# SimonsRoad/gf-pl-slam

Hardware: AMD Instinct MI355X
Metric: stereo frames/sec (2k ORB + 500 LBD, 10 GN iters) (higher is better)
Workload: dtype f64

## Files before the change

### gf-pl-slam_amd/csrc/gfpl_abi.hip

```cpp
#include <hip/hip_runtime.h>

#include <algorithm>
#include <atomic>
#include <cmath>
#include <mutex>
#include <cstdio>
#include <cstdlib>
#include <cstring>
#include <vector>

#include "../../include/gfpl.h"
#include "gfpl_kernels.hpp"

using namespace gfpl;

#define GFPL_NEV 10

struct gfpl_ctx {
    int device = 0;
    hipStream_t stream = nullptr;
    bool own_stream = false;
    gfpl_camera cam{};
    gfpl_config cfg{};
    bool has_cam = false, has_cfg = false;
    bool timing = false;
    hipEvent_t ev[GFPL_NEV]{};
    float stage_ms[7]{};
    std::vector<gfpl_seqbatch*> sbs;
    std::atomic<int> n_detectors{0};
    std::mutex host_mu;
    char* fuse_ws = nullptr;
    size_t fuse_ws_bytes = 0;
    int* fuse_host = nullptr;
    hipEvent_t fuse_ev[2][4]{};
    bool fuse_timed[2] = {false, false};
};

struct gfpl_seqbatch {
    gfpl_ctx* ctx = nullptr;
    int B = 0, kp_cap = 0, kl_cap = 0, mpt_cap = 0, mls_cap = 0;
    void* base = nullptr;
    int64_t bytes = 0;
    DevFrame slot[2];
    int prev_slot = 0;
    bool initialized = false;
    bool has_curr = false;
    DevTrack tr{};
    DevScratch scr{};
    void* stage[2] = {nullptr, nullptr};
    size_t stage_bytes[2] = {0, 0};
    gfpl_frames stage_view[2]{};
    hipStream_t copy = nullptr;
    hipEvent_t ev_ready[2]{}, ev_free[2]{};
    bool ready_pending[2] = {false, false}, free_recorded[2] = {false, false};
    hipEvent_t ev_ticket[16]{};
    int64_t n_tickets = 0;
    int32_t* last_n_pt = nullptr;
    int32_t* last_n_ls = nullptr;
    PyrBuild* pyrb = nullptr;
    int last_cut_mode = -1;
};

struct gfpl_event {
    int device = 0;
    hipEvent_t ev = nullptr;
    int64_t records = 0;
};

int gfpl_ctx_device(const gfpl_ctx* c) { return c->device; }
void* gfpl_ctx_stream(const gfpl_ctx* c) { return (void*)c->stream; }
const gfpl_camera* gfpl_ctx_camera(const gfpl_ctx* c) { return c->has_cam ? &c->cam : nullptr; }
const gfpl_config* gfpl_ctx_config(const gfpl_ctx* c) { return &c->cfg; }
int64_t gfpl_event_records(const gfpl_event* e) { return e->records; }
void gfpl_ctx_attach(gfpl_ctx* c) { c->n_detectors.fetch_add(1); }
void gfpl_ctx_detach(gfpl_ctx* c) { c->n_detectors.fetch_sub(1); }


namespace {

#define HIPCHK(x)                                                  \
    do {                                                            \
        hipError_t e_ = (x);                                        \
        if (e_ != hipSuccess) {                                     \
            std::fprintf(stderr, "gfpl: %s failed: %s\n", #x, hipGetErrorString(e_)); \
            return GFPL_E_HIP;                                      \
        }                                                           \
    } while (0)

int debug_fill_byte() { return env_int("GFPL_DEBUG_FILL", 0) & 0xFF; }

template <typename F, typename H, typename V>
void frame_fields(F& f, H& o, V& v) {
    v.pt(f.pt.pl, o.pt_pl, 2); v.pt(f.pt.pl_obs, o.pt_pl_obs, 2);
    v.pt(f.pt.disp, o.pt_disp, 1); v.pt(f.pt.P, o.pt_P, 3); v.pt(f.pt.sigma2, o.pt_sigma2, 1);
    v.pt(f.pt.idx, o.pt_idx, 1); v.pt(f.pt.level, o.pt_level, 1); v.pt(f.pt.inlier, o.pt_inlier, 1);
    v.pt(f.pt.desc, o.pdesc, 32); v.count(f.pt.n);
    v.ls(f.ls.spl, o.ls_spl, 2); v.ls(f.ls.epl, o.ls_epl, 2);
    v.ls(f.ls.spl_obs, o.ls_spl_obs, 2); v.ls(f.ls.epl_obs, o.ls_epl_obs, 2);
    v.ls(f.ls.sdisp, o.ls_sdisp, 1); v.ls(f.ls.edisp, o.ls_edisp, 1);
    v.ls(f.ls.sdisp_obs, o.ls_sdisp_obs, 1); v.ls(f.ls.edisp_obs, o.ls_edisp_obs, 1);
    v.ls(f.ls.angle, o.ls_angle, 1); v.ls(f.ls.sigma2, o.ls_sigma2, 1);
    v.ls(f.ls.sP, o.ls_sP, 3); v.ls(f.ls.eP, o.ls_eP, 3);
    v.ls(f.ls.le, o.ls_le, 3); v.ls(f.ls.le_obs, o.ls_le_obs, 3);
    v.ls(f.ls.covS, o.ls_covS, 9); v.ls(f.ls.covE, o.ls_covE, 9);
    v.ls(f.ls.cut, o.ls_cut, 2); v.ls(f.ls.invcov, o.ls_invcov, 36);
    v.ls(f.ls.idx, o.ls_idx, 1); v.ls(f.ls.level, o.ls_level, 1); v.ls(f.ls.inlier, o.ls_inlier, 1);
    v.ls(f.ls.desc, o.ldesc, 32); v.count(f.ls.n);
    v.seq(f.pose.Tfw, o.Tfw, 16); v.seq(f.pose.DT, o.DT, 16);
    v.seq(f.pose.DT_cov, o.DT_cov, 36); v.seq(f.pose.Tfw_cov, o.Tfw_cov, 36);
    v.seq(f.pose.DT_cov_eig, o.DT_cov_eig, 6);
    v.seq(f.pose.err_norm, &o.err_norm, 1); v.seq(f.pose.time_stamp, &o.time_stamp, 1);
}

struct SlotCarve {
    Carver& c;
    size_t B, P, L;
    template <typename T, typename U> void pt(T*& d, U, int w) { d = c.take<T>(P * w); }
    template <typename T, typename U> void ls(T*& d, U, int w) { d = c.take<T>(L * w); }
    template <typename T, typename U> void seq(T*& d, U, int w) { d = c.take<T>(B * w); }
    void count(int32_t*& d) { d = c.take<int32_t>(B); }
};

void carve(Carver& c, gfpl_seqbatch* sb) {
    const size_t B = sb->B, P = (size_t)B * sb->kp_cap, L = (size_t)B * sb->kl_cap;
    const gfpl_frame_host none{};
    SlotCarve v{c, B, P, L};
    for (int s = 0; s < 2; ++s) frame_fields(sb->slot[s], none, v);
    sb->tr.matched_pt = c.take<int32_t>(B * sb->mpt_cap);
    sb->tr.n_matched_pt = c.take<int32_t>(B);
    sb->tr.matched_ls = c.take<int32_t>(B * sb->mls_cap);
    sb->tr.n_matched_ls = c.take<int32_t>(B);
    sb->tr.n_inliers = c.take<int32_t>(B);
    sb->tr.n_inliers_pt = c.take<int32_t>(B);
    sb->tr.n_inliers_ls = c.take<int32_t>(B);
    sb->tr.num_frame_loss = c.take<int32_t>(B);
    sb->tr.kf_T = c.take<double>(B * 16);
    sb->tr.kf_cov = c.take<double>(B * 36);
    sb->tr.kf_entropy0 = c.take<double>(B);
    sb->tr.kf_ratio = c.take<double>(B);
    sb->tr.kf_prev_iskf = c.take<int32_t>(B);
    sb->tr.kf_nsince = c.take<int32_t>(B);
    sb->tr.kf_flag = c.take<int32_t>(B);
    sb->scr.cut_rec = c.take<double>(B * sb->mls_cap * CUT_REC);
    sb->scr.knn = c.take<int32_t>(B * 2 * (size_t)sb->kp_cap * 3);
    sb->scr.proj = reinterpret_cast<double*>(sb->scr.knn);
    sb->scr.bytes = c.take<int64_t>(B * STEP_REC);
    sb->scr.n_subpix = c.take<int32_t>(B);
    sb->scr.cut_sum = c.take<double>(B * CUT_SUM_REC);
    sb->scr.cut_dtinv = c.take<double>(B * 16);
    sb->scr.cut_vtab = c.take<double>(B * sb->mls_cap * 2 * CUT_KS);
    sb->scr.pose_DT = c.take<double>(B * 16);
    sb->scr.pose_H = c.take<double>(B * 36);
    sb->scr.pose_err = c.take<double>(B);
    sb->scr.pose_ok = c.take<int32_t>(B);
    sb->scr.pose_in = c.take<double>(B * (6 * (size_t)sb->mpt_cap + 10 * (size_t)sb->mls_cap));
    sb->scr.pose_act = c.take<double>(B * (6 * (size_t)sb->mpt_cap + 10 * (size_t)sb->mls_cap));
    sb->scr.pose_dtini = c.take<double>(B * 16);
    sb->scr.cross_tinv = c.take<double>(B * 16);
    sb->scr.dbg = c.take<int64_t>(B * DBG_REC);
    sb->scr.cut_prog = c.take<int32_t>((size_t)1 << 17);
    sb->scr.cut_path = c.take<uint8_t>(B * sb->mls_cap * CUT_PATH);
    sb->scr.cut_flag = c.take<int32_t>(B);
    sb->scr.cut_vmax = c.take<double>(B * sb->mls_cap * CUT_VMAX);
    sb->scr.cut_offl = c.take<int32_t>(1 + B * sb->mls_cap);
    sb->scr.cut_dtln = c.take<int32_t>(1 + CUT_DTL * B);
    sb->scr.cut_dtl = c.take<double>(CUT_DTL * B * CUT_DTL_REC);
    sb->scr.kf_mask = c.take<int32_t>(B);
    sb->last_n_pt = c.take<int32_t>(B);
    sb->last_n_ls = c.take<int32_t>(B);
}

DevCam devcam(const gfpl_camera& c) {
    DevCam d;
    d.fx = c.fx; d.fy = c.fy; d.cx = c.cx; d.cy = c.cy; d.b = c.b;
    d.width = c.width; d.height = c.height; d.n_levels = c.n_levels;
    for (int i = 0; i < GFPL_MAX_LEVELS; ++i) {
        d.scale[i] = c.scale[i]; d.inv_scale[i] = c.inv_scale[i];
        d.lvl_cols[i] = c.lvl_cols[i]; d.lvl_rows[i] = c.lvl_rows[i];
        d.lvl_offset[i] = c.lvl_offset[i];
        d.sigma2_pt[i] = c.sigma2_pt[i]; d.sigma2_ln[i] = c.sigma2_ln[i];
    }
    d.pyr_bytes = c.pyr_bytes;
    return d;
}

KParams params(gfpl_seqbatch* sb, const gfpl_frames* in) {
    KParams p;
    std::memset(&p, 0, sizeof p);
    p.cam = devcam(sb->ctx->cam);
    p.cfg = sb->ctx->cfg;
    p.prev = sb->slot[sb->prev_slot];
    p.curr = sb->slot[1 - sb->prev_slot];
    p.tr = sb->tr;
    p.scr = sb->scr;
    if (in) p.in = *in;
    p.B = sb->B; p.kp_cap = sb->kp_cap; p.kl_cap = sb->kl_cap;
    p.mpt_cap = sb->mpt_cap; p.mls_cap = sb->mls_cap;
    p.cfg.max_point_match_num = std::min(p.cfg.max_point_match_num, sb->mpt_cap);
    p.cfg.max_line_match_num = std::min(p.cfg.max_line_match_num, sb->mls_cap);
    p.sp_maxD = (float)p.cam.fx;
    p.sp_mbf = (float)(p.cam.fx * p.cam.b);
    p.cut_tq = 0.25 * p.cfg.cut_certify - 4.0 * 0x1p-53;
    {
        const double s = p.cfg.cut_step, lo = p.cfg.cut_rng[0], hi = p.cfg.cut_rng[1];
        auto same = [](double x, double y) { return std::memcmp(&x, &y, sizeof x) == 0; };
        int n = 0;
        for (double t = 0.0; n < CUT_KS && t <= hi && s > 0.0; t = t + s) p.cut_keys[n++] = t;
        const int ns = n;
        for (int i = 1; i < ns && n < CUT_KS; ++i) {
            const double e = p.cut_keys[i] - s;
            bool have = false;
            for (int k = 0; k < n; ++k) have = have || same(p.cut_keys[k], e);
            if (!have && e >= lo) p.cut_keys[n++] = e;
        }
        for (int i = 0; i < n; ++i) {
            int up = -1, dn = -1;
            for (int k = 0; k < n; ++k) {
                if (same(p.cut_keys[k], p.cut_keys[i] + s)) up = k;
                if (same(p.cut_keys[k], p.cut_keys[i] - s)) dn = k;
            }
            p.cut_knxt[i] = (int8_t)up;
            p.cut_kprv[i] = (int8_t)dn;
        }
        p.cut_nkeys = n;
    }
    return p;
}

int check_in(gfpl_seqbatch* sb, const gfpl_frames* in) {
    if (!in) return GFPL_E_INVALID;
    if (in->batch != sb->B || in->kp_cap != sb->kp_cap || in->kl_cap != sb->kl_cap) return GFPL_E_INVALID;
    if (!in->n_kp_l || !in->n_kp_r || !in->kp_l || !in->kp_r || !in->pdesc_l || !in->pdesc_r || !in->n_kl_l ||
        !in->n_kl_r || !in->kl_l || !in->kl_r || !in->ldesc_l || !in->ldesc_r || !in->pyr_r || !in->time_stamp)
        return GFPL_E_INVALID;
    if (((uintptr_t)in->pyr_r & 3) != 0) return GFPL_E_INVALID;
    if ((in->ready && in->ready->device != sb->ctx->device) || (in->consumed && in->consumed->device != sb->ctx->device))
        return GFPL_E_INVALID;
    return GFPL_OK;
}

int in_acquire(gfpl_seqbatch* sb, const gfpl_frames* in) {
    if (in->ready && hipStreamWaitEvent(sb->ctx->stream, in->ready->ev, 0) != hipSuccess) return -2;
    for (int s = 0; s < 2; ++s)
        if (sb->stage[s] && in->n_kp_l == sb->stage_view[s].n_kp_l) {
            if (sb->ready_pending[s] && hipStreamWaitEvent(sb->ctx->stream, sb->ev_ready[s], 0) != hipSuccess) return -2;
            return s;
        }
    return -1;
}
int in_release(gfpl_seqbatch* sb, const gfpl_frames* in, int slot) {
    if (in->consumed) {
        if (hipEventRecord(in->consumed->ev, sb->ctx->stream) != hipSuccess) return GFPL_E_HIP;
        ++in->consumed->records;
    }
    if (slot < 0) return GFPL_OK;
    if (hipEventRecord(sb->ev_free[slot], sb->ctx->stream) != hipSuccess) return GFPL_E_HIP;
    sb->free_recorded[slot] = true;
    return GFPL_OK;
}

static int cut_mode(const gfpl_config& c) { return c.cut_with_max_vol ? c.cut_proof : 0; }

int cfg_supported(const gfpl_config& c) {
    if (!c.best_lr_matches || !c.lr_in_parallel) return GFPL_E_UNSUPPORTED;
    if (c.max_point_match_num < 1 || c.max_point_match_num > GFPL_MAX_MATCHED_PT) return GFPL_E_INVALID;
    if (c.max_line_match_num < 1 || c.max_line_match_num > GFPL_MAX_MATCHED_LS) return GFPL_E_INVALID;
    if (!(c.cut_certify == 0.0 || (c.cut_certify >= 1e-10 && c.cut_certify < 1.0))) return GFPL_E_INVALID;
    if (c.cut_proof < 0 || c.cut_proof > 3) return GFPL_E_INVALID;
// ... 139 lines not shown
    if (e) return e;
    for (const gfpl_seqbatch* sb : c->sbs)
        if (cfg->max_point_match_num > sb->mpt_cap || cfg->max_line_match_num > sb->mls_cap) return GFPL_E_CAPACITY;
    c->cfg = *cfg;
    c->has_cfg = true;
    return GFPL_OK;
}

int gfpl_get_camera(const gfpl_ctx* c, gfpl_camera* cam) {
    if (!c || !cam || !c->has_cam) return GFPL_E_INVALID;
    *cam = c->cam;
    return GFPL_OK;
}

int gfpl_get_config(const gfpl_ctx* c, gfpl_config* cfg) {
    if (!c || !cfg) return GFPL_E_INVALID;
    *cfg = c->cfg;
    return GFPL_OK;
}

int gfpl_synchronize(gfpl_ctx* c) {
    if (!c) return GFPL_E_INVALID;
    HIPCHK(hipStreamSynchronize(c->stream));
    return GFPL_OK;
}

int gfpl_seqbatch_create(gfpl_ctx* c, int batch, int kp_cap, int kl_cap, gfpl_seqbatch** out) {
    if (!c || !out || batch < 1 || kp_cap < 2 || kl_cap < 2 || kp_cap > 8192 || kl_cap > 2048 || !c->has_cam)
        return GFPL_E_INVALID;
    HIPCHK(hipSetDevice(c->device));
    gfpl_seqbatch* sb = new gfpl_seqbatch();
    sb->ctx = c;
    sb->B = batch;
    sb->kp_cap = (kp_cap + 1) & ~1;
    sb->kl_cap = (kl_cap + 1) & ~1;
    sb->mpt_cap = c->cfg.max_point_match_num;
    sb->mls_cap = c->cfg.max_line_match_num;
    Carver dry;
    carve(dry, sb);
    sb->bytes = (int64_t)dry.off;
    if (hipMalloc(&sb->base, dry.off) != hipSuccess) { delete sb; return GFPL_E_HIP; }
    if (hipMemsetAsync(sb->base, debug_fill_byte(), dry.off, c->stream) != hipSuccess) { (void)hipFree(sb->base); delete sb; return GFPL_E_HIP; }
    Carver real;
    real.base = (char*)sb->base;
    carve(real, sb);
    if (sb->kp_cap != kp_cap || sb->kl_cap != kl_cap) {
        (void)hipFree(sb->base); delete sb; return GFPL_E_INVALID;
    }
    c->sbs.push_back(sb);
    *out = sb;
    return GFPL_OK;
}

int gfpl_seqbatch_destroy(gfpl_seqbatch* sb) {
    if (!sb) return GFPL_E_INVALID;
    (void)hipStreamSynchronize(sb->ctx->stream);
    auto& v = sb->ctx->sbs;
    v.erase(std::remove(v.begin(), v.end(), sb), v.end());
    if (sb->copy) (void)hipStreamSynchronize(sb->copy);
    if (sb->base) (void)hipFree(sb->base);
    for (int k = 0; k < 2; ++k) {
        if (sb->stage[k]) (void)hipFree(sb->stage[k]);
        if (sb->ev_ready[k]) (void)hipEventDestroy(sb->ev_ready[k]);
        if (sb->ev_free[k]) (void)hipEventDestroy(sb->ev_free[k]);
    }
    for (hipEvent_t e : sb->ev_ticket)
        if (e) (void)hipEventDestroy(e);
    if (sb->copy) (void)hipStreamDestroy(sb->copy);
    pyrbuild_destroy(sb->pyrb);
    delete sb;
    return GFPL_OK;
}

int64_t gfpl_seqbatch_bytes(const gfpl_seqbatch* sb) { return sb ? sb->bytes : 0; }

int gfpl_initialize(gfpl_seqbatch* sb, const gfpl_frames* in) {
    if (!sb) return GFPL_E_INVALID;
    int e = check_in(sb, in);
    if (e) return e;
    const int slot = in_acquire(sb, in);
    if (slot == -2) return GFPL_E_HIP;
    KParams p = params(sb, in);
    p.curr = sb->slot[sb->prev_slot];
    HIPCHK(launch_init(p, sb->ctx->stream));
    sb->initialized = true;
    sb->has_curr = false;
    return in_release(sb, in, slot);
}

int gfpl_stereo_points(gfpl_seqbatch* sb, const gfpl_frames* in) {
    if (!sb) return GFPL_E_INVALID;
    if (!sb->initialized) return GFPL_E_STATE;
    int e = check_in(sb, in);
    if (e) return e;
    const int slot = in_acquire(sb, in);
    if (slot == -2) return GFPL_E_HIP;
    HIPCHK(launch_stereo_points(params(sb, in), sb->ctx->stream));
    sb->has_curr = true;
    return in_release(sb, in, slot);
}

int gfpl_stereo_lines(gfpl_seqbatch* sb, const gfpl_frames* in) {
    if (!sb) return GFPL_E_INVALID;
    if (!sb->initialized) return GFPL_E_STATE;
    int e = check_in(sb, in);
    if (e) return e;
    const int slot = in_acquire(sb, in);
    if (slot == -2) return GFPL_E_HIP;
    HIPCHK(launch_stereo_lines(params(sb, in), sb->ctx->stream));
    sb->has_curr = true;
    return in_release(sb, in, slot);
}

int gfpl_line_uncertainty(gfpl_seqbatch* sb) {
    if (!sb) return GFPL_E_INVALID;
    if (!sb->initialized) return GFPL_E_STATE;
    HIPCHK(launch_line_uncertainty(params(sb, nullptr), sb->ctx->stream));
    return GFPL_OK;
}

int gfpl_cross_points(gfpl_seqbatch* sb) {
    if (!sb) return GFPL_E_INVALID;
    if (!sb->initialized || !sb->has_curr) return GFPL_E_STATE;
    HIPCHK(launch_cross_points(params(sb, nullptr), sb->ctx->stream));
    return GFPL_OK;
}

int gfpl_cross_lines(gfpl_seqbatch* sb) {
    if (!sb) return GFPL_E_INVALID;
    if (!sb->initialized || !sb->has_curr) return GFPL_E_STATE;
    HIPCHK(launch_cross_lines(params(sb, nullptr), sb->ctx->stream));
    return GFPL_OK;
}

int gfpl_line_cut(gfpl_seqbatch* sb) {
    if (!sb) return GFPL_E_INVALID;
    if (!sb->initialized || !sb->has_curr) return GFPL_E_STATE;
    sb->last_cut_mode = cut_mode(sb->ctx->cfg);
    HIPCHK(launch_line_cut(params(sb, nullptr), sb->ctx->stream, nullptr));
    return GFPL_OK;
}

int gfpl_insert_stereo_pair(gfpl_seqbatch* sb, const gfpl_frames* in) {
    if (!sb) return GFPL_E_INVALID;
    if (!sb->initialized) return GFPL_E_STATE;
    int e = check_in(sb, in);
    if (e) return e;
    gfpl_ctx* c = sb->ctx;
    const int slot = in_acquire(sb, in);
    if (slot == -2) return GFPL_E_HIP;
    KParams p = params(sb, in);
    tmark(c, 0);
    HIPCHK(launch_stereo_points(p, c->stream));
    tmark(c, 1);
    HIPCHK(launch_stereo_lines(p, c->stream));
    tmark(c, 2);
    if (c->cfg.use_line_conf_cut) HIPCHK(launch_line_uncertainty(p, c->stream));
    HIPCHK(launch_cross_points(p, c->stream));
    tmark(c, 3);
    HIPCHK(launch_cross_lines(p, c->stream));
    tmark(c, 4);
    sb->last_cut_mode = c->cfg.use_line_conf_cut ? cut_mode(c->cfg) : -1;
    if (c->cfg.use_line_conf_cut)
        HIPCHK(launch_line_cut(p, c->stream, c->timing ? &c->ev[7] : nullptr));
    HIPCHK(launch_step_bytes(p, c->stream));
    tmark(c, 5);
    sb->has_curr = true;
    return in_release(sb, in, slot);
}

int gfpl_optimize_pose(gfpl_seqbatch* sb) {
    if (!sb) return GFPL_E_INVALID;
    if (!sb->initialized || !sb->has_curr) return GFPL_E_STATE;
    HIPCHK(launch_pose(params(sb, nullptr), sb->ctx->stream, sb->ctx->timing ? sb->ctx->ev[9] : nullptr));
    tmark(sb->ctx, 6);
    return GFPL_OK;
}

int gfpl_need_new_kf(gfpl_seqbatch* sb, int32_t* flags) {
    if (!sb) return GFPL_E_INVALID;
    if (!sb->initialized || !sb->has_curr) return GFPL_E_STATE;
    HIPCHK(launch_need_kf(params(sb, nullptr), sb->ctx->stream));
    if (flags) {
        HIPCHK(hipMemcpyAsync(flags, sb->tr.kf_flag, sizeof(int32_t) * (size_t)sb->B, hipMemcpyDeviceToHost,
                              sb->ctx->stream));
        HIPCHK(hipStreamSynchronize(sb->ctx->stream));
    }
    return GFPL_OK;
}

int gfpl_curr_frame_is_kf(gfpl_seqbatch* sb, const int32_t* mask) {
    if (!sb) return GFPL_E_INVALID;
    if (!sb->initialized || !sb->has_curr) return GFPL_E_STATE;
    const int32_t* dmask = sb->tr.kf_flag;
    if (mask) {
        HIPCHK(hipMemcpyAsync(sb->scr.kf_mask, mask, sizeof(int32_t) * (size_t)sb->B, hipMemcpyHostToDevice,
                              sb->ctx->stream));
        dmask = sb->scr.kf_mask;
    }
    HIPCHK(launch_curr_frame_is_kf(params(sb, nullptr), dmask, sb->ctx->stream));
    if (mask) HIPCHK(hipStreamSynchronize(sb->ctx->stream));
    return GFPL_OK;
}

int gfpl_read_kf_state(gfpl_seqbatch* sb, int seq, gfpl_kf_state* out) {
    if (!sb || !out || seq < 0 || seq >= sb->B) return GFPL_E_INVALID;
    hipStream_t s = sb->ctx->stream;
    const DevTrack& T = sb->tr;
    HIPCHK(hipMemcpyAsync(out->T_prevKF, T.kf_T + 16 * (size_t)seq, sizeof(double) * 16, hipMemcpyDeviceToHost, s));
    HIPCHK(hipMemcpyAsync(out->cov_prevKF_currF, T.kf_cov + 36 * (size_t)seq, sizeof(double) * 36,
                          hipMemcpyDeviceToHost, s));
    HIPCHK(hipMemcpyAsync(&out->entropy_first_prevKF, T.kf_entropy0 + seq, sizeof(double), hipMemcpyDeviceToHost, s));
    HIPCHK(hipMemcpyAsync(&out->entropy_ratio, T.kf_ratio + seq, sizeof(double), hipMemcpyDeviceToHost, s));
    HIPCHK(hipMemcpyAsync(&out->prev_f_iskf, T.kf_prev_iskf + seq, sizeof(int32_t), hipMemcpyDeviceToHost, s));
    HIPCHK(hipMemcpyAsync(&out->num_frame_since_kf, T.kf_nsince + seq, sizeof(int32_t), hipMemcpyDeviceToHost, s));
    HIPCHK(hipMemcpyAsync(&out->need_new_kf, T.kf_flag + seq, sizeof(int32_t), hipMemcpyDeviceToHost, s));
    HIPCHK(hipStreamSynchronize(s));
    return GFPL_OK;
}

int gfpl_optimize_pose_ini(gfpl_seqbatch* sb, const double* dt_ini) {
    if (!sb) return GFPL_E_INVALID;
    if (!dt_ini) return gfpl_optimize_pose(sb);
    if (!sb->initialized || !sb->has_curr) return GFPL_E_STATE;
    HIPCHK(hipMemcpyAsync(sb->scr.pose_dtini, dt_ini, sizeof(double) * 16 * (size_t)sb->B, hipMemcpyHostToDevice,
                          sb->ctx->stream));
    KParams p = params(sb, nullptr);
    p.dt_ini = sb->scr.pose_dtini;
    HIPCHK(launch_pose(p, sb->ctx->stream, sb->ctx->timing ? sb->ctx->ev[9] : nullptr));
    tmark(sb->ctx, 6);
    HIPCHK(hipStreamSynchronize(sb->ctx->stream));
    return GFPL_OK;
}

}

namespace {
void stage_layout(Carver& c, const gfpl_seqbatch* sb, gfpl_frames& f) {
    const size_t B = sb->B, P = B * sb->kp_cap, L = B * sb->kl_cap;
    const size_t pyr = B * (size_t)sb->ctx->cam.pyr_bytes;
    f.batch = sb->B; f.kp_cap = sb->kp_cap; f.kl_cap = sb->kl_cap;
    f.n_kp_l = c.take<int>(B); f.n_kp_r = c.take<int>(B);
    f.kp_l = c.take<gfpl_keypoint>(P); f.kp_r = c.take<gfpl_keypoint>(P);
    f.pdesc_l = c.take<uint8_t>(P * 32); f.pdesc_r = c.take<uint8_t>(P * 32);
    f.n_kl_l = c.take<int>(B); f.n_kl_r = c.take<int>(B);
    f.kl_l = c.take<gfpl_keyline>(L); f.kl_r = c.take<gfpl_keyline>(L);
    f.ldesc_l = c.take<uint8_t>(L * 32); f.ldesc_r = c.take<uint8_t>(L * 32);
// ... 47 lines not shown
}

}

namespace {
int upload_async(gfpl_seqbatch* sb, const gfpl_frames* host, int s0, int slot, int64_t l0_stride, int64_t* ticket) {
    if (!sb || !host || (slot != 0 && slot != 1) || !sb->ctx->has_cam) return GFPL_E_INVALID;
    const int n = host->batch;
    if (n < 1 || s0 < 0 || s0 + n > sb->B || host->kp_cap != sb->kp_cap || host->kl_cap != sb->kl_cap)
        return GFPL_E_INVALID;
    if (!host->n_kp_l || !host->n_kp_r || !host->kp_l || !host->kp_r || !host->pdesc_l || !host->pdesc_r ||
        !host->n_kl_l || !host->n_kl_r || !host->kl_l || !host->kl_r || !host->ldesc_l || !host->ldesc_r ||
        !host->pyr_r || !host->time_stamp)
        return GFPL_E_INVALID;
    int e = stage_alloc(sb, slot);
    if (e) return e;
    const gfpl_frames& d = sb->stage_view[slot];
    hipStream_t s = sb->copy;
    if (sb->free_recorded[slot]) HIPCHK(hipStreamWaitEvent(s, sb->ev_free[slot], 0));
    const size_t N = n, P = N * sb->kp_cap, L = N * sb->kl_cap, S = s0;
    const size_t kp0 = S * sb->kp_cap, kl0 = S * sb->kl_cap, pyr = (size_t)sb->ctx->cam.pyr_bytes;
#define UP(field, off, cnt) \
    HIPCHK(hipMemcpyAsync((void*)(d.field + (off)), host->field, sizeof(*d.field) * (cnt), hipMemcpyHostToDevice, s))
    UP(n_kp_l, S, N); UP(n_kp_r, S, N); UP(kp_l, kp0, P); UP(kp_r, kp0, P);
    UP(pdesc_l, kp0 * 32, P * 32); UP(pdesc_r, kp0 * 32, P * 32);
    UP(n_kl_l, S, N); UP(n_kl_r, S, N); UP(kl_l, kl0, L); UP(kl_r, kl0, L);
    UP(ldesc_l, kl0 * 32, L * 32); UP(ldesc_r, kl0 * 32, L * 32);
    UP(time_stamp, S, N);
    if (l0_stride > 0) {
        const gfpl_camera& cam = sb->ctx->cam;
        const size_t l0 = (size_t)cam.lvl_cols[0] * cam.lvl_rows[0];
        uint8_t* dst = const_cast<uint8_t*>(d.pyr_r) + S * pyr;
        HIPCHK(hipMemcpy2DAsync(dst, pyr, host->pyr_r, (size_t)l0_stride, l0, N, hipMemcpyHostToDevice, s));
        HIPCHK(pyrbuild_run(sb->pyrb, dst, (long long)pyr, n, s));
    } else {
        UP(pyr_r, S * pyr, N * pyr);
    }
#undef UP
    HIPCHK(hipEventRecord(sb->ev_ready[slot], s));
    sb->ready_pending[slot] = true;
    const int64_t t = sb->n_tickets++;
    HIPCHK(hipEventRecord(sb->ev_ticket[t % 16], s));
    if (ticket) *ticket = t;
    return GFPL_OK;
}
}

extern "C" {

int gfpl_upload_wait(gfpl_seqbatch* sb, int64_t ticket) {
    if (!sb || ticket < 0 || ticket >= sb->n_tickets) return GFPL_E_INVALID;
    HIPCHK(hipEventSynchronize(sb->ev_ticket[ticket % 16]));
    return GFPL_OK;
}

int gfpl_staged_frames(gfpl_seqbatch* sb, int slot, gfpl_frames* dev) {
    if (!sb || !dev || (slot != 0 && slot != 1) || !sb->stage[slot]) return GFPL_E_INVALID;
    *dev = sb->stage_view[slot];
    return GFPL_OK;
}

int gfpl_upload_frames(gfpl_seqbatch* sb, const gfpl_frames* host, gfpl_frames* dev) {
    if (!sb || !host || !dev) return GFPL_E_INVALID;
    if (host->batch != sb->B) return GFPL_E_INVALID;
    int64_t t = 0;
    int e = gfpl_upload_frames_async(sb, host, 0, 0, &t);
    if (e) return e;
    e = gfpl_upload_wait(sb, t);
    if (e) return e;
    *dev = sb->stage_view[0];
    return GFPL_OK;
}

int gfpl_update_frame(gfpl_seqbatch* sb) {
    if (!sb) return GFPL_E_INVALID;
    if (!sb->initialized || !sb->has_curr) return GFPL_E_STATE;
    HIPCHK(hipMemcpyAsync(sb->last_n_pt, sb->tr.n_matched_pt, sizeof(int32_t) * sb->B, hipMemcpyDeviceToDevice,
                          sb->ctx->stream));
    HIPCHK(hipMemcpyAsync(sb->last_n_ls, sb->tr.n_matched_ls, sizeof(int32_t) * sb->B, hipMemcpyDeviceToDevice,
                          sb->ctx->stream));
    HIPCHK(hipMemsetAsync(sb->tr.n_matched_pt, 0, sizeof(int32_t) * sb->B, sb->ctx->stream));
    HIPCHK(hipMemsetAsync(sb->tr.n_matched_ls, 0, sizeof(int32_t) * sb->B, sb->ctx->stream));
    sb->prev_slot = 1 - sb->prev_slot;
    sb->has_curr = false;
    return GFPL_OK;
}

int gfpl_frame_step(gfpl_seqbatch* sb, const gfpl_frames* in) {
    int e = gfpl_insert_stereo_pair(sb, in);
    if (e) return e;
    e = gfpl_optimize_pose(sb);
    if (e) return e;
    return gfpl_update_frame(sb);
}

int gfpl_knn2_hamming(gfpl_ctx* c, const uint8_t* q, int nq, const uint8_t* t, int nt, int cell, int32_t* idx,
                      float* dist) {
    if (!c || !q || !t || !idx || !dist || nq < 0 || (cell != 1 && cell != 2)) return GFPL_E_INVALID;
    if (nt < 2) return GFPL_E_TOO_FEW_TRAIN;
    if (nq == 0) return GFPL_OK;
    HIPCHK(launch_knn2(q, nq, t, nt, cell, idx, dist, c->stream));
    return GFPL_OK;
}

namespace {
struct Scratch {
    char* p = nullptr;
    ~Scratch() { if (p) (void)hipFree(p); }
};
inline bool misaligned16(const void* p) { return (reinterpret_cast<uintptr_t>(p) & 15) != 0; }
}

int gfpl_knn2_hamming_host(gfpl_ctx* c, const uint8_t* q, int nq, const uint8_t* t, int nt, int cell, int32_t* idx,
                           float* dist) {
    if (!c || !q || !t || !idx || !dist || nq < 0 || (cell != 1 && cell != 2)) return GFPL_E_INVALID;
    if (nt < 2) return GFPL_E_TOO_FEW_TRAIN;
    if (nq == 0) return GFPL_OK;
    std::lock_guard<std::mutex> lk(c->host_mu);
    HIPCHK(hipSetDevice(c->device));
    const size_t bq = 32 * (size_t)nq, bt = 32 * (size_t)nt, bo = 2 * (size_t)nq * 4;
    Scratch s;
    HIPCHK(hipMalloc(&s.p, bq + bt + 2 * bo + 64));
    uint8_t* dq = reinterpret_cast<uint8_t*>(s.p);
    uint8_t* dt = dq + bq;
    int32_t* di = reinterpret_cast<int32_t*>(dt + bt);
    float* dd = reinterpret_cast<float*>(di + 2 * (size_t)nq);
    HIPCHK(hipMemcpyAsync(dq, q, bq, hipMemcpyHostToDevice, c->stream));
    HIPCHK(hipMemcpyAsync(dt, t, bt, hipMemcpyHostToDevice, c->stream));
    HIPCHK(launch_knn2(dq, nq, dt, nt, cell, di, dd, c->stream));
    HIPCHK(hipMemcpyAsync(idx, di, bo, hipMemcpyDeviceToHost, c->stream));
    HIPCHK(hipMemcpyAsync(dist, dd, bo, hipMemcpyDeviceToHost, c->stream));
    HIPCHK(hipStreamSynchronize(c->stream));
    return GFPL_OK;
}

int gfpl_radius_hamming(gfpl_ctx* c, const uint8_t* q, int nq, const uint8_t* t, int nt, int cell, float max_dist,
                        int32_t* row_off, int cap, int32_t* idx, float* dist) {
    if (!c || (!q && nq) || (!t && nt) || !row_off || nq < 0 || nt < 0 || cap < 0 || (cell != 1 && cell != 2) ||
        max_dist != max_dist)
        return GFPL_E_INVALID;
    HIPCHK(hipSetDevice(c->device));
    std::vector<int32_t> h(nq + 1, 0);
    if (nq > 0 && nt > 0) {
        HIPCHK(launch_radius_count(q, nq, t, nt, cell, max_dist, row_off + 1, c->stream));
        HIPCHK(hipMemcpyAsync(h.data() + 1, row_off + 1, 4 * (size_t)nq, hipMemcpyDeviceToHost, c->stream));
        HIPCHK(hipStreamSynchronize(c->stream));
    }
    for (int i = 0; i < nq; ++i) h[i + 1] += h[i];
    HIPCHK(hipMemcpyAsync(row_off, h.data(), 4 * (size_t)(nq + 1), hipMemcpyHostToDevice, c->stream));
    HIPCHK(hipStreamSynchronize(c->stream));
    if (h[nq] > cap) return GFPL_E_CAPACITY;
    if (h[nq] > 0) {
        if (!idx || !dist) return GFPL_E_INVALID;
        HIPCHK(launch_radius_rows(q, nq, t, nt, cell, max_dist, row_off, idx, dist, c->stream));
    }
    HIPCHK(hipStreamSynchronize(c->stream));
    return GFPL_OK;
}

int gfpl_radius_hamming_host(gfpl_ctx* c, const uint8_t* q, int nq, const uint8_t* t, int nt, int cell, float max_dist,
                             int32_t* row_off, int cap, int32_t* idx, float* dist) {
    if (!c || (!q && nq) || (!t && nt) || !row_off || nq < 0 || nt < 0 || cap < 0 || (cell != 1 && cell != 2) ||
        max_dist != max_dist)
        return GFPL_E_INVALID;
    std::lock_guard<std::mutex> lk(c->host_mu);
    HIPCHK(hipSetDevice(c->device));
// ... 387 lines not shown
        la.out = d_res;
        e = launch_loop_closure(la, n, c->stream);
    }
    if (e == hipSuccess)
        e = hipMemcpyAsync(out, d_res, (size_t)n * sizeof(gfpl_loop_result), hipMemcpyDeviceToHost, c->stream);
    hipError_t es = hipStreamSynchronize(c->stream);
    hipError_t ef = hipFree(scr);
    if (e != hipSuccess || es != hipSuccess || ef != hipSuccess) return GFPL_E_HIP;
    return GFPL_OK;
}

}

namespace {
template <typename T>
hipError_t d2h(T* dst, const T* src, size_t n, hipStream_t s) {
    if (!dst || n == 0) return hipSuccess;
    return hipMemcpyAsync(dst, src, n * sizeof(T), hipMemcpyDeviceToHost, s);
}
template <typename T>
hipError_t h2d(T* dst, const T* src, size_t n, hipStream_t s) {
    if (!src || n == 0) return hipSuccess;
    return hipMemcpyAsync(dst, src, n * sizeof(T), hipMemcpyHostToDevice, s);
}
#define XFER(fn, a, b, n) HIPCHK(fn(a, b, n, s))

template <bool READ>
struct SlotCopy {
    hipStream_t s;
    size_t b, P, L, np, nl;
    hipError_t e = hipSuccess;
    template <typename T, typename U>
    void rows(T* d, U* h, size_t off, size_t n) {
        if (e != hipSuccess) return;
        if constexpr (READ) e = d2h(h, d + off, n, s);
        else e = h2d(d + off, h, n, s);
    }
    template <typename T, typename U> void pt(T* d, U* h, int w) { rows(d, h, w * P, w * np); }
    template <typename T, typename U> void ls(T* d, U* h, int w) { rows(d, h, w * L, w * nl); }
    template <typename T, typename U> void seq(T* d, U* h, int w) { rows(d, h, w * b, (size_t)w); }
    void count(int32_t*) {}
};

int read_track(gfpl_seqbatch* sb, int seq, gfpl_track_host* o, const int32_t* n_pt, const int32_t* n_ls) {
    if (!sb || !o || seq < 0 || seq >= sb->B) return GFPL_E_INVALID;
    hipStream_t s = sb->ctx->stream;
    HIPCHK(hipStreamSynchronize(s));
    std::memset(o, 0, sizeof(*o));
    XFER(d2h, &o->n_matched_pt, n_pt + seq, 1);
    XFER(d2h, &o->n_matched_ls, n_ls + seq, 1);
    XFER(d2h, &o->n_inliers, sb->tr.n_inliers + seq, 1);
    XFER(d2h, &o->n_inliers_pt, sb->tr.n_inliers_pt + seq, 1);
    XFER(d2h, &o->n_inliers_ls, sb->tr.n_inliers_ls + seq, 1);
    XFER(d2h, &o->num_frame_loss, sb->tr.num_frame_loss + seq, 1);
    HIPCHK(hipStreamSynchronize(s));
    XFER(d2h, o->matched_pt, sb->tr.matched_pt + (size_t)seq * sb->mpt_cap, (size_t)o->n_matched_pt);
    XFER(d2h, o->matched_ls, sb->tr.matched_ls + (size_t)seq * sb->mls_cap, (size_t)o->n_matched_ls);
    HIPCHK(hipStreamSynchronize(s));
    return GFPL_OK;
}
}

extern "C" {

int gfpl_read_frame(gfpl_seqbatch* sb, int which, int seq, gfpl_frame_host* o) {
    if (!sb || !o || seq < 0 || seq >= sb->B || (which != GFPL_PREV && which != GFPL_CURR)) return GFPL_E_INVALID;
    hipStream_t s = sb->ctx->stream;
    const DevFrame& f = sb->slot[which == GFPL_PREV ? sb->prev_slot : 1 - sb->prev_slot];
    HIPCHK(hipStreamSynchronize(s));
    int np = 0, nl = 0;
    HIPCHK(hipMemcpy(&np, f.pt.n + seq, 4, hipMemcpyDeviceToHost));
    HIPCHK(hipMemcpy(&nl, f.ls.n + seq, 4, hipMemcpyDeviceToHost));
    o->n_pt = np; o->n_ls = nl;
    SlotCopy<true> v{s, (size_t)seq, (size_t)seq * sb->kp_cap, (size_t)seq * sb->kl_cap, (size_t)np, (size_t)nl};
    frame_fields(f, *o, v);
    HIPCHK(v.e);
    HIPCHK(hipStreamSynchronize(s));
    return GFPL_OK;
}

int gfpl_write_frame(gfpl_seqbatch* sb, int which, int seq, const gfpl_frame_host* o) {
    if (!sb || !o || seq < 0 || seq >= sb->B || (which != GFPL_PREV && which != GFPL_CURR)) return GFPL_E_INVALID;
    if (o->n_pt < 0 || o->n_pt > sb->kp_cap || o->n_ls < 0 || o->n_ls > sb->kl_cap) return GFPL_E_CAPACITY;
    hipStream_t s = sb->ctx->stream;
    const DevFrame& f = sb->slot[which == GFPL_PREV ? sb->prev_slot : 1 - sb->prev_slot];
    XFER(h2d, f.pt.n + seq, &o->n_pt, 1);
    XFER(h2d, f.ls.n + seq, &o->n_ls, 1);
    SlotCopy<false> v{s, (size_t)seq, (size_t)seq * sb->kp_cap, (size_t)seq * sb->kl_cap, (size_t)o->n_pt, (size_t)o->n_ls};
    frame_fields(f, *o, v);
    HIPCHK(v.e);
    HIPCHK(hipStreamSynchronize(s));
    sb->initialized = true;
    if (which == GFPL_CURR) sb->has_curr = true;
    return GFPL_OK;
}

int gfpl_read_track(gfpl_seqbatch* sb, int seq, gfpl_track_host* o) {
    return read_track(sb, seq, o, sb ? sb->tr.n_matched_pt : nullptr, sb ? sb->tr.n_matched_ls : nullptr);
}

int gfpl_read_last_track(gfpl_seqbatch* sb, int seq, gfpl_track_host* o) {
    return read_track(sb, seq, o, sb ? sb->last_n_pt : nullptr, sb ? sb->last_n_ls : nullptr);
}

int gfpl_write_track(gfpl_seqbatch* sb, int seq, const gfpl_track_host* o) {
    if (!sb || !o || seq < 0 || seq >= sb->B) return GFPL_E_INVALID;
    if (o->n_matched_pt < 0 || o->n_matched_pt > sb->mpt_cap || o->n_matched_ls < 0 || o->n_matched_ls > sb->mls_cap)
        return GFPL_E_CAPACITY;
    for (int i = 0; i < o->n_matched_pt; ++i)
        if (o->matched_pt[i] < 0 || o->matched_pt[i] >= sb->kp_cap) return GFPL_E_INVALID;
    for (int i = 0; i < o->n_matched_ls; ++i)
        if (o->matched_ls[i] < 0 || o->matched_ls[i] >= sb->kl_cap) return GFPL_E_INVALID;
    hipStream_t s = sb->ctx->stream;
    XFER(h2d, sb->tr.n_matched_pt + seq, &o->n_matched_pt, 1);
    XFER(h2d, sb->tr.n_matched_ls + seq, &o->n_matched_ls, 1);
    XFER(h2d, sb->tr.n_inliers + seq, &o->n_inliers, 1);
    XFER(h2d, sb->tr.n_inliers_pt + seq, &o->n_inliers_pt, 1);
    XFER(h2d, sb->tr.n_inliers_ls + seq, &o->n_inliers_ls, 1);
    XFER(h2d, sb->tr.num_frame_loss + seq, &o->num_frame_loss, 1);
    XFER(h2d, sb->tr.matched_pt + (size_t)seq * sb->mpt_cap, o->matched_pt, (size_t)o->n_matched_pt);
    XFER(h2d, sb->tr.matched_ls + (size_t)seq * sb->mls_cap, o->matched_ls, (size_t)o->n_matched_ls);
    HIPCHK(hipStreamSynchronize(s));
    return GFPL_OK;
}

int gfpl_set_timing(gfpl_ctx* c, int enable) {
    if (!c) return GFPL_E_INVALID;
    c->timing = enable != 0;
    return GFPL_OK;
}

int gfpl_get_stage_times(gfpl_ctx* c, float* ms7) {
    if (!c || !ms7) return GFPL_E_INVALID;
    if (!c->timing) return GFPL_E_STATE;
    HIPCHK(hipEventSynchronize(c->ev[6]));
    for (int i = 0; i < 6; ++i) HIPCHK(hipEventElapsedTime(&ms7[i], c->ev[i], c->ev[i + 1]));
    HIPCHK(hipEventElapsedTime(&ms7[6], c->ev[0], c->ev[6]));
    return GFPL_OK;
}

int gfpl_get_kernel_times(gfpl_ctx* c, float* ms4) {
    if (!c || !ms4) return GFPL_E_INVALID;
    if (!c->timing) return GFPL_E_STATE;
    if (!c->cfg.use_line_conf_cut) return GFPL_E_STATE;
    HIPCHK(hipEventSynchronize(c->ev[6]));
    HIPCHK(hipEventElapsedTime(&ms4[0], c->ev[4], c->ev[7]));
    HIPCHK(hipEventElapsedTime(&ms4[1], c->ev[7], c->ev[8]));
    HIPCHK(hipEventElapsedTime(&ms4[2], c->ev[8], c->ev[5]));
    HIPCHK(hipEventElapsedTime(&ms4[3], c->ev[5], c->ev[9]));
    return GFPL_OK;
}

}

namespace {
int step_rec_sums(gfpl_seqbatch* sb, int64_t* sums) {
    std::vector<int64_t> v((size_t)sb->B * STEP_REC);
    HIPCHK(hipStreamSynchronize(sb->ctx->stream));
    HIPCHK(hipMemcpy(v.data(), sb->scr.bytes, sizeof(int64_t) * v.size(), hipMemcpyDeviceToHost));
    for (int s = 0; s < STEP_REC; ++s) {
        int64_t t = 0;
        for (int b = 0; b < sb->B; ++b) t += v[(size_t)b * STEP_REC + s];
        sums[s] = t;
    }
    return GFPL_OK;
}
int step_rec_sums(gfpl_seqbatch* sb, int first, int n, int64_t* out, bool on = true) {
    if (!sb || !out) return GFPL_E_INVALID;
    int64_t v[STEP_REC];
    const int e = step_rec_sums(sb, v);
    if (e) return e;
    for (int s = 0; s < n; ++s) out[s] = on ? v[first + s] : 0;
    return GFPL_OK;
}
}

extern "C" {

int gfpl_last_step_kernel_bytes(gfpl_seqbatch* sb, int64_t* bytes4) {
    if (!sb || !bytes4) return GFPL_E_INVALID;
    int64_t v[STEP_REC];
    int e = step_rec_sums(sb, v);
    if (e) return e;
    const bool cut = sb->last_cut_mode >= 0;
    bytes4[0] = cut ? 212 * v[GFPL_STEP_M_L] + 44 * v[GFPL_STEP_M_P] + 552 * (int64_t)sb->B : 0;
    bytes4[1] = v[GFPL_STEP_B_CUT_SEARCH];
    bytes4[2] = cut ? 612 * v[GFPL_STEP_M_L] : 0;
    bytes4[3] = v[GFPL_STEP_B_POSE];
    return GFPL_OK;
}

int gfpl_last_step_stage_bytes(gfpl_seqbatch* sb, int64_t* bytes7) {
    return step_rec_sums(sb, GFPL_STEP_B_STEREO_POINTS, 7, bytes7);
}

int gfpl_last_step_counts(gfpl_seqbatch* sb, int64_t* counts8) {
    return step_rec_sums(sb, GFPL_STEP_N_O, 8, counts8);
}

int gfpl_last_step_track_counts(gfpl_seqbatch* sb, int64_t* counts4) {
    return step_rec_sums(sb, GFPL_STEP_CUT_STEPS, 4, counts4);
}

int gfpl_last_step_cut_proof(gfpl_seqbatch* sb, int64_t* counts4) {
    return step_rec_sums(sb, GFPL_STEP_PROOF_REDONE, 4, counts4,
                         sb && (sb->last_cut_mode == 1 || sb->last_cut_mode == 3));
}

int gfpl_debug_cut_records(gfpl_seqbatch* sb, int b, double* out, int n_lines) {
    if (!sb || !out || b < 0 || b >= sb->B || n_lines < 0 || n_lines > sb->mls_cap) return GFPL_E_INVALID;
    if (hipSetDevice(sb->ctx->device) != hipSuccess) return GFPL_E_HIP;
    if (hipStreamSynchronize(sb->ctx->stream) != hipSuccess) return GFPL_E_HIP;
    const size_t n = (size_t)n_lines * CUT_REC;
    return hipMemcpy(out, sb->scr.cut_rec + (size_t)b * sb->mls_cap * CUT_REC, n * sizeof(double),
                     hipMemcpyDeviceToHost) == hipSuccess ? GFPL_OK : GFPL_E_HIP;
}

int gfpl_debug_step_records(gfpl_seqbatch* sb, int64_t* out) {
    if (!sb || !out) return GFPL_E_INVALID;
    if (hipSetDevice(sb->ctx->device) != hipSuccess) return GFPL_E_HIP;
    if (hipStreamSynchronize(sb->ctx->stream) != hipSuccess) return GFPL_E_HIP;
    return hipMemcpy(out, sb->scr.bytes, (size_t)sb->B * STEP_REC * sizeof(int64_t), hipMemcpyDeviceToHost) == hipSuccess
               ? GFPL_OK : GFPL_E_HIP;
}

int gfpl_debug_clocks(gfpl_seqbatch* sb, int64_t* out) {
    if (!sb || !out) return GFPL_E_INVALID;
    if (hipSetDevice(sb->ctx->device) != hipSuccess) return GFPL_E_HIP;
    if (hipStreamSynchronize(sb->ctx->stream) != hipSuccess) return GFPL_E_HIP;
    return hipMemcpy(out, sb->scr.dbg, (size_t)sb->B * DBG_REC * sizeof(int64_t), hipMemcpyDeviceToHost) == hipSuccess
               ? GFPL_OK : GFPL_E_HIP;
}

int gfpl_last_step_bytes(gfpl_seqbatch* sb, int64_t* bytes) {
    if (!bytes) return GFPL_E_INVALID;
    return step_rec_sums(sb, GFPL_STEP_B_TOTAL, 1, bytes);
}

}
```

### gf-pl-slam_amd/csrc/gfpl_device.hpp

```cpp
#pragma once
#include <hip/hip_runtime.h>
#include <stdint.h>

#include "../../include/gfpl.h"

#define GFPL_DEV __device__ __forceinline__

namespace gfpl {

GFPL_DEV uint32_t hiw(double x) { return (uint32_t)((uint64_t)__double_as_longlong(x) >> 32); }
GFPL_DEV uint32_t low(double x) { return (uint32_t)(uint64_t)__double_as_longlong(x); }
GFPL_DEV double with_hi(double x, uint32_t hi) {
    uint64_t u = (uint64_t)__double_as_longlong(x);
    u = ((uint64_t)hi << 32) | (u & 0xffffffffull);
    return __longlong_as_double((long long)u);
}
GFPL_DEV double from_words(uint32_t hi, uint32_t lo) {
    return __longlong_as_double((long long)(((uint64_t)hi << 32) | lo));
}

GFPL_DEV double det_log(double x) {
    const double ln2_hi = 6.93147180369123816490e-01, ln2_lo = 1.90821492927058770002e-10,
                 two54 = 1.80143985094819840000e+16,
                 Lg1 = 6.666666666666735130e-01, Lg2 = 3.999999999940941908e-01,
// ... 775 lines not shown
    uv[0] = c.cx + (c.fx * P[0]) / P[2];
    uv[1] = c.cy + (c.fy * P[1]) / P[2];
}
GFPL_DEV void backProjection(const DevCam& c, double u, double v, double disp, double* P) {
    double bd = c.b / disp;
    P[0] = bd * (u - c.cx);
    P[1] = bd * (v - c.cy);
    P[2] = bd * c.fx;
}

struct SharedDiv { double b, sb, r; };
GFPL_DEV double div_refine(double sb) {
    double r = __builtin_amdgcn_rcp(sb);
    double t = __builtin_fma(-sb, r, 1.0);
    r = __builtin_fma(r, t, r);
    t = __builtin_fma(-sb, r, 1.0);
    return __builtin_fma(r, t, r);
}
GFPL_DEV SharedDiv div_prep(double b, double a0) {
    bool f;
    const double sb = __builtin_amdgcn_div_scale(a0, b, false, &f);
    return SharedDiv{b, sb, div_refine(sb)};
}
GFPL_DEV double div_by(const SharedDiv& d, double a) {
    bool f, vcc;
    const double sb = __builtin_amdgcn_div_scale(a, d.b, false, &f);
    double r = d.r;
    if (__builtin_expect(__double_as_longlong(sb) != __double_as_longlong(d.sb), 0)) r = div_refine(sb);
    const double sa = __builtin_amdgcn_div_scale(a, d.b, true, &vcc);
    const double m = sa * r;
    const double e = __builtin_fma(-sb, m, sa);
    return __builtin_amdgcn_div_fixup(__builtin_amdgcn_div_fmas(e, r, m, vcc), d.b, a);
}
template <typename T>
GFPL_DEV void poseJac_t(const DevCam& c, double homog, const T* g, T lx, T ly, T* J) {
    T gx = g[0], gy = g[1], gz = g[2];
    T gz2 = gz * gz;
    T fgz2 = T(c.fx) / ref_max(homog, gz2);
    J[0] = (fgz2 * lx) * gz;
    J[1] = (fgz2 * ly) * gz;
    J[2] = (-fgz2) * ((gx * lx) + (gy * ly));
    J[3] = (-fgz2) * ((((gx * gy) * lx) + ((gy * gy) * ly)) + ((gz * gz) * ly));
    J[4] = fgz2 * ((((gx * gx) * lx) + ((gz * gz) * lx)) + ((gx * gy) * ly));
    J[5] = fgz2 * (((gx * gz) * ly) - ((gy * gz) * lx));
}
GFPL_DEV void poseJac(const DevCam& c, double homog, const double* g, double lx, double ly, double* J) {
    poseJac_t<double>(c, homog, g, lx, ly, J);
}

GFPL_DEV void endpointCov(const DevCam& cam, double u, double v, double disp, double* C) {
    double f = cam.fx;
    double px = u - cam.cx, py = v - cam.cy;
    double d2 = disp * disp;
    C[0] = d2 + (2.0 * px) * px;
    C[1] = (2.0 * px) * py;
    C[2] = (2.0 * f) * px;
    C[4] = d2 + (2.0 * py) * py;
    C[5] = (2.0 * f) * py;
    C[8] = (2.0 * f) * f;
    C[3] = C[1]; C[6] = C[2]; C[7] = C[5];
    double dd = d2 * d2;
#pragma unroll
    for (int i = 0; i < 9; ++i) C[i] = ((C[i] * cam.b) * cam.b) / dd;
}

GFPL_DEV void covMat2D_3D(const DevCam& cam, double u, double v, double u_std, double d, double d_std, double* cov) {
    double cov2D[9] = {u_std * u_std, 0, 0, 0, u_std * u_std, 0, 0, 0, d_std * d_std};
    double b = cam.b, d_2 = d * d;
    double J[9];
    J[0] = b / d; J[3] = 0.0; J[6] = 0.0;
    J[1] = 0.0; J[4] = b / d; J[7] = 0.0;
    J[2] = ((-(u - cam.cx)) * b) / d_2;
    J[5] = ((-(v - cam.cy)) * b) / d_2;
    J[8] = ((-cam.fx) * b) / d_2;
    double JC[9];
    mat3_mul(J, cov2D, JC);
#pragma unroll
    for (int i = 0; i < 3; ++i)
#pragma unroll
        for (int j = 0; j < 3; ++j)
            cov[i * 3 + j] = (JC[i * 3 + 0] * J[j * 3 + 0] + JC[i * 3 + 1] * J[j * 3 + 1]) + JC[i * 3 + 2] * J[j * 3 + 2];
}

GFPL_DEV double std_min(double a, double b) { return (b < a) ? b : a; }
GFPL_DEV double std_max(double a, double b) { return (a < b) ? b : a; }
GFPL_DEV double overlapStereo(double spl_obs, double epl_obs, double spl_proj, double epl_proj) {
    double sln = std_min(spl_obs, epl_obs);
    double eln = std_max(spl_obs, epl_obs);
    double spn = std_min(spl_proj, epl_proj);
    double epn = std_max(spl_proj, epl_proj);
    double length = eln - spn;
    double overlap;
    if ((epn < sln) || (spn > eln)) overlap = 0.0;
    else {
        if ((epn > eln) && (spn < sln)) overlap = eln - sln;
        else overlap = std_min(eln, epn) - std_max(sln, spn);
    }
    if (length > 0.01f) overlap = overlap / length;
    else overlap = 0.0;
    return overlap;
}

__device__ __forceinline__ int wave_hist_rank(const int* h, int r, int nb) {
    const int lane = threadIdx.x & 63;
    int loc[5], sum = 0;
#pragma unroll
    for (int i = 0; i < 5; ++i) {
        const int v = lane * 5 + i;
        loc[i] = v < nb ? h[v] : 0;
        sum += loc[i];
    }
    int inc = sum;
#pragma unroll
    for (int o = 1; o < 64; o <<= 1) {
        const int y = __shfl_up(inc, o, 64);
        if (lane >= o) inc += y;
    }
    int res = 0x7FFFFFFF;
    if (inc - sum <= r && r < inc) {
        int c = inc - sum;
#pragma unroll
        for (int i = 0; i < 5; ++i) {
            c += loc[i];
            if (c > r && res == 0x7FFFFFFF) res = lane * 5 + i;
        }
    }
#pragma unroll
    for (int o = 32; o > 0; o >>= 1) res = min(res, __shfl_xor(res, o, 64));
    return res == 0x7FFFFFFF ? nb - 1 : res;
}

template <int BLOCK>
GFPL_DEV int block_exclusive_scan(int v, int* lds , int* total) {
    const int lane = threadIdx.x & 63, wid = threadIdx.x >> 6;
    int x = v;
#pragma unroll
    for (int o = 1; o < 64; o <<= 1) {
        int y = __shfl_up(x, o, 64);
        if (lane >= o) x += y;
    }
    if (lane == 63) lds[wid] = x;
    __syncthreads();
    if (threadIdx.x == 0) {
        int s = 0;
        for (int w = 0; w < BLOCK / 64; ++w) { int t = lds[w]; lds[w] = s; s += t; }
        lds[BLOCK / 64] = s;
    }
    __syncthreads();
    int r = x - v + lds[wid];
    *total = lds[BLOCK / 64];
    __syncthreads();
    return r;
}

template <int BLOCK>
GFPL_DEV int scan_tiles(int32_t* tile, int nt, int* scan) {
    int carry = 0;
    for (int b0 = 0; b0 < nt; b0 += BLOCK) {
        const int b = b0 + threadIdx.x;
        const int v = b < nt ? tile[b] : 0;
        int total;
        const int ex = block_exclusive_scan<BLOCK>(v, scan, &total);
        if (b < nt) tile[b] = carry + ex;
        carry += total;
    }
    if (threadIdx.x == 0) tile[nt] = carry;
// ... 35 lines not shown
```

### gf-pl-slam_amd/csrc/gfpl_kernels.hpp

```cpp
#pragma once
#include "gfpl_layout.hpp"
#include "gfpl_state.hpp"

#include <atomic>
#include <cstdlib>

namespace gfpl {

inline int env_int(const char* name, int dflt) {
    const char* e = getenv(name);
    if (!e) return dflt;
    return (int)strtol(e, nullptr, (e[0] == '0' && (e[1] == 'x' || e[1] == 'X')) ? 16 : 10);
}

inline hipError_t ensure_dyn_lds(const void* fn, int bytes, std::atomic<unsigned long long>* done) {
    int dev = 0;
    hipError_t e = hipGetDevice(&dev);
    if (e != hipSuccess) return e;
    const unsigned long long bit = dev < 64 ? 1ull << dev : 0ull;
    if (bit && (done->load(std::memory_order_acquire) & bit)) return hipSuccess;
    e = hipFuncSetAttribute(fn, hipFuncAttributeMaxDynamicSharedMemorySize, bytes);
    if (e == hipSuccess && bit) done->fetch_or(bit, std::memory_order_acq_rel);
    return e;
}

constexpr int DYN_LDS_CEILING = 160 * 1024 - 1024;

int sp_wide_max_b();
hipError_t launch_stereo_points(const KParams& p, hipStream_t s);
hipError_t launch_stereo_lines(const KParams& p, hipStream_t s);
hipError_t launch_line_uncertainty(const KParams& p, hipStream_t s);
hipError_t launch_init(const KParams& p, hipStream_t s);
hipError_t launch_knn2(const uint8_t* q, int nq, const uint8_t* t, int nt, int cell, int32_t* idx, float* dist,
                       hipStream_t s);
hipError_t launch_knn2_batched(const uint8_t* q, const int* nq, const uint8_t* t, const int* nt, int cap, int B,
                               int cell, int32_t* packed, hipStream_t s);
hipError_t launch_knn2_counts(const uint8_t* q, const int* nq, const uint8_t* t, const int* nt, int cap, int cell,
                              int32_t* idx, float* dist, hipStream_t s);
hipError_t launch_radius_count(const uint8_t* q, int nq, const uint8_t* t, int nt, int cell, float radius,
                               int32_t* cnt, hipStream_t s);
hipError_t launch_radius_rows(const uint8_t* q, int nq, const uint8_t* t, int nt, int cell, float radius,
                              const int32_t* row_off, int32_t* idx, float* dist, hipStream_t s);
hipError_t launch_match_stats(int kind, const float* d0, const float* d1, int n, int max_num, double* out,
                              hipStream_t s);
hipError_t launch_cross_points(const KParams& p, hipStream_t s);
hipError_t launch_cross_lines(const KParams& p, hipStream_t s);
hipError_t launch_line_cut(const KParams& p, hipStream_t s, const hipEvent_t* marks );
hipError_t launch_pose(const KParams& p, hipStream_t s, hipEvent_t mark );
hipError_t launch_step_bytes(const KParams& p, hipStream_t s);
hipError_t launch_need_kf(const KParams& p, hipStream_t s);
hipError_t launch_curr_frame_is_kf(const KParams& p, const int32_t* mask , hipStream_t s);

struct KfGate {
    DevCam cam;
    double T0[16], T1[16];
    double max_ratio_12_p, desc_th_l;
    int lines, n0;
    int map;
    const int32_t* loc;
    int p_stride;
    double epip_p, epip_l;
    const double* le1;
    const int32_t* i12;
    const float* d12;
    const int32_t* i21;
    const double* P0;
    const double* eP0;
    const double* le0;
    const double* sigma2_0;
    const double* pl1;
    int32_t* pairs;
    int* count;
};
hipError_t launch_kf_gate(const KfGate& g, hipStream_t s);
hipError_t launch_kf_map_filter(const DevCam& cam, const double* T1, const double* P, int n, int lines,
                                int32_t* loc, uint8_t* desc_out, const uint8_t* desc_in, int* count, hipStream_t s);

struct FuseSelect {
    DevCam cam;
    int lines, n, n_kf;
    const double* X;
    const int32_t* kf;
    const double* T_kf;
    const uint8_t* desc_in;
    int32_t* loc;
    uint8_t* desc_out;
    int* count;
    int* bad_kf;
};
struct FuseGate {
    int lines, cap;
    const int* n_sel;
    const int32_t* loc;
    const int32_t* idx;
    const double* X;
    double max_pp, max_pl, max_dl;
    int32_t* pairs;
    int* count;
};
hipError_t launch_fuse_select(const FuseSelect& a, hipStream_t s);
hipError_t launch_fuse_gate(const FuseGate& g, hipStream_t s);

struct LoopPair {
    int n0_pt, n0_ls;
    const int32_t *pi12, *pi21;
    const int32_t *li12, *li21;
    const double* P0;
    const double* pl1;
    const double *sP0, *eP0;
    const double* le1;
};
struct LoopArgs {
    DevCam cam;
    double homog_th;
    int max_iters;
    gfpl_loop_params prm;
    const LoopPair* pairs;
    int pt_cap, ls_cap;
    int32_t* pt_pairs;
    uint8_t* pt_inlier;
    int32_t* ls_pairs;
    uint8_t* ls_inlier;
    gfpl_loop_result* out;
};
hipError_t launch_loop_closure(const LoopArgs& a, int n, hipStream_t s);

struct BowVocabDev {
    const uint8_t* desc;
    const BowNode* node;
    const int32_t* rank_word;
// ... 231 lines not shown
```

### gf-pl-slam_amd/csrc/k_cut.hip

```cpp
#include "gfpl_kernels.hpp"
#include "gfpl_wave.hpp"

namespace gfpl {

struct LineCutData {
    double sP[3], eP[3], covS[9], covE[9], Jl[2];
};

template <typename T, bool SD = false>
__device__ __forceinline__ T endpointVar_t(const DevCam& cam, const double* DT_inv, const T* Jl, const T* Pt,
                                           const T* cov, double zlo) {
    T Jdt[9];
#pragma unroll
    for (int i = 0; i < 3; ++i)
#pragma unroll
        for (int j = 0; j < 3; ++j) Jdt[i * 3 + j] = T(DT_inv[i * 4 + j]);
    T cur[3];
    se3_apply_t<T, double>(DT_inv, Pt, cur);
    rb_floor(cur[2], zlo);
    const T f = T(cam.fx), pz = cur[2], pz_2 = pz * pz;
    T Jp[9];
    Jp[0] = f / pz; Jp[3] = T(0.0); Jp[6] = T(0.0);
    Jp[1] = T(0.0); Jp[4] = f / pz; Jp[7] = T(0.0);
    if constexpr (SD) {
// ... 23 lines not shown
#pragma unroll
        for (int j = 0; j < 3; ++j)
            T3[i * 3 + j] = (T2[i * 3 + 0] * Jdt[j * 3 + 0] + T2[i * 3 + 1] * Jdt[j * 3 + 1]) + T2[i * 3 + 2] * Jdt[j * 3 + 2];
#pragma unroll
    for (int i = 0; i < 2; ++i)
#pragma unroll
        for (int j = 0; j < 2; ++j)
            M[i * 2 + j] = (T3[i * 3 + 0] * Jp[j * 3 + 0] + T3[i * 3 + 1] * Jp[j * 3 + 1]) + T3[i * 3 + 2] * Jp[j * 3 + 2];
    const T r0 = Jl[0] * M[0] + Jl[1] * M[2];
    const T r1 = Jl[0] * M[1] + Jl[1] * M[3];
    return r0 * Jl[0] + r1 * Jl[1];
}

template <typename T, bool VAR = true>
__device__ __forceinline__ void cut_endpoint_t(const DevCam& cam, double homog, const double* DT_inv, const T* Jl,
                                               const T* P0, const T* P1, const T* C0, const T* C1, T c, T* out7,
                                               double zlo) {
    T Pt[3];
#pragma unroll
    for (int k = 0; k < 3; ++k) Pt[k] = (T(1.0) - c) * P0[k] + c * P1[k];
    if (VAR) {
        const T a = (T(1.0) - c) * (T(1.0) - c), q = c * c;
        T cov[9];
#pragma unroll
        for (int i = 0; i < 9; ++i) cov[i] = a * C0[i] + q * C1[i];
        out7[0] = endpointVar_t<T>(cam, DT_inv, Jl, Pt, cov, zlo);
    }
    T cur[3];
    se3_apply_t<T, double>(DT_inv, Pt, cur);
    rb_floor(cur[2], zlo);
    poseJac_t<T>(cam, homog, cur, Jl[0], Jl[1], out7 + 1);
}
__device__ __forceinline__ void cut_endpoint(const DevCam& cam, double homog, const double* DT_inv, const double* Jl,
                                             const double* P0, const double* P1, const double* C0, const double* C1,
                                             double c, double* out7) {
    cut_endpoint_t<double>(cam, homog, DT_inv, Jl, P0, P1, C0, C1, c, out7, 0.0);
}

template <bool FULL>
__device__ __forceinline__ void cut_assemble(const double* S7, const double* E7, double* info) {
    const double vs = S7[0], ve = E7[0];
    const double* Js = S7 + 1;
    const double* Je = E7 + 1;
    const double det = vs * ve - 0.0 * 0.0;
    const double invdet = 1.0 / det;
    const double i00 = ve * invdet, i10 = -0.0 * invdet, i01 = -0.0 * invdet, i11 = vs * invdet;
    double T0[6], T1[6];
#pragma unroll
    for (int i = 0; i < 6; ++i) {
        T0[i] = Js[i] * i00 + Je[i] * i10;
        T1[i] = Js[i] * i01 + Je[i] * i11;
    }
    if (FULL) {
#pragma unroll
        for (int i = 0; i < 6; ++i)
#pragma unroll
            for (int j = 0; j < 6; ++j) info[i * 6 + j] = T0[i] * Js[j] + T1[i] * Je[j];
    } else {
#pragma unroll
        for (int i = 0; i < 6; ++i)
#pragma unroll
            for (int j = 0; j <= i; ++j) info[tri(i, j)] = T0[i] * Js[j] + T1[i] * Je[j];
    }
}

template <bool FULL>
__device__ __forceinline__ void poseInfoOnLine(const DevCam& cam, double homog, const double* DT_inv,
                                               const LineCutData& L, double c0, double c1, double* info) {
    double S7[7], E7[7];
    cut_endpoint(cam, homog, DT_inv, L.Jl, L.sP, L.eP, L.covS, L.covE, c0, S7);
    cut_endpoint(cam, homog, DT_inv, L.Jl, L.eP, L.sP, L.covE, L.covS, c1, E7);
    cut_assemble<FULL>(S7, E7, info);
}

__device__ __forceinline__ void load_line(const DevLines& L, size_t q, LineCutData& d) {
#pragma unroll
    for (int k = 0; k < 3; ++k) { d.sP[k] = L.sP[3 * q + k]; d.eP[k] = L.eP[3 * q + k]; }
#pragma unroll
    for (int k = 0; k < 9; ++k) { d.covS[k] = L.covS[9 * q + k]; d.covE[k] = L.covE[9 * q + k]; }
    d.Jl[0] = L.le_obs[3 * q];
    d.Jl[1] = L.le_obs[3 * q + 1];
}


template <typename T>
__device__ __forceinline__ T sym3_t(const T* A, const T* x, const T* y) {
    const T ax = (A[0] * y[0] + A[1] * y[1]) + A[2] * y[2];
    const T ay = (A[1] * y[0] + A[3] * y[1]) + A[4] * y[2];
    const T az = (A[2] * y[0] + A[4] * y[1]) + A[5] * y[2];
    return (x[0] * ax + x[1] * ay) + x[2] * az;
}

template <typename T>
__device__ __forceinline__ void cut_poly_coeff_t(const T* g0, const T* g1, T lx, T ly, int k, T* Pk) {
    const T dx = g1[0] - g0[0], dy = g1[1] - g0[1], dz = g1[2] - g0[2];
    auto prod = [&](T a0, T a1, T b0, T b1) -> T {
        return k == 0 ? a0 * b0 : (k == 1 ? a0 * b1 + a1 * b0 : a1 * b1);
    };
    auto lin = [&](T a0, T a1) -> T { return k == 0 ? a0 : (k == 1 ? a1 : T(0.0)); };
    const T x0 = g0[0], y0 = g0[1], z0 = g0[2];
    Pk[0] = lx * lin(z0, dz);
    Pk[1] = ly * lin(z0, dz);
    Pk[2] = -(lx * lin(x0, dx) + ly * lin(y0, dy));
    Pk[3] = -((lx * prod(x0, dx, y0, dy) + ly * prod(y0, dy, y0, dy)) + ly * prod(z0, dz, z0, dz));
    Pk[4] = (lx * prod(x0, dx, x0, dx) + lx * prod(z0, dz, z0, dz)) + ly * prod(x0, dx, y0, dy);
    Pk[5] = ly * prod(x0, dx, z0, dz) - lx * prod(y0, dy, z0, dz);
}

template <typename T>
__device__ __forceinline__ void cut_poly_coef_t(const double* Dl, const T* sP, const T* eP, const T* covS,
                                                const T* covE, const T* Jl, T* P, T* V, T* g) {
    se3_apply_t<T, double>(Dl, sP, g);
    se3_apply_t<T, double>(Dl, eP, g + 3);
    T A[2][6];
    const T* Cs[2] = {covS, covE};
#pragma unroll
    for (int w = 0; w < 2; ++w) {
        T Tm[9];
#pragma unroll
        for (int i = 0; i < 3; ++i)
#pragma unroll
            for (int k = 0; k < 3; ++k)
                Tm[i * 3 + k] = (T(Dl[i * 4 + 0]) * Cs[w][0 * 3 + k] + T(Dl[i * 4 + 1]) * Cs[w][1 * 3 + k]) +
                                T(Dl[i * 4 + 2]) * Cs[w][2 * 3 + k];
        const int ii[6] = {0, 0, 0, 1, 1, 2}, jj[6] = {0, 1, 2, 1, 2, 2};
#pragma unroll
        for (int e = 0; e < 6; ++e)
            A[w][e] = (Tm[ii[e] * 3 + 0] * T(Dl[jj[e] * 4 + 0]) + Tm[ii[e] * 3 + 1] * T(Dl[jj[e] * 4 + 1])) +
                      Tm[ii[e] * 3 + 2] * T(Dl[jj[e] * 4 + 2]);
    }
#pragma unroll
    for (int side = 0; side < 2; ++side) {
        T* Ps = P + 18 * side;
#pragma unroll
        for (int k = 0; k < 3; ++k) cut_poly_coeff_t<T>(g + 3 * side, g + 3 * (1 - side), Jl[0], Jl[1], k, Ps + 6 * k);
        const T* p0 = Ps;
        const T* p1 = Ps + 6;
        const T a0 = sym3_t<T>(A[side], p0, p0), a1 = sym3_t<T>(A[side], p0, p1), a2 = sym3_t<T>(A[side], p1, p1);
        const T b0 = sym3_t<T>(A[1 - side], p0, p0), b1 = sym3_t<T>(A[1 - side], p0, p1), b2 = sym3_t<T>(A[1 - side], p1, p1);
        T* v = V + 5 * side;
        v[0] = a0;
        v[1] = T(2.0) * (a1 - a0);
        v[2] = ((a2 - T(4.0) * a1) + a0) + b0;
        v[3] = T(2.0) * ((a1 - a2) + b1);
        v[4] = a2 + b2;
    }
}

__device__ __forceinline__ void cut_poly_data(const double* Dl, const LineCutData& d, double homog, double* fd) {
    double P[36], V[10], g[6];
    cut_poly_coef_t<double>(Dl, d.sP, d.eP, d.covS, d.covE, d.Jl, P, V, g);
#pragma unroll
    for (int i = 0; i < 18; ++i) { fd[PD_PS + i] = P[i]; fd[PD_PE + i] = P[18 + i]; }
#pragma unroll
    for (int i = 0; i < 5; ++i) { fd[PD_VS + i] = V[i]; fd[PD_VE + i] = V[5 + i]; }
    const double z0 = g[2], z1 = g[5];
    fd[PD_OK] = (((z0 > 0.0 && z1 > 0.0) || (z0 < 0.0 && z1 < 0.0)) && z0 * z0 > 2.0 * homog && z1 * z1 > 2.0 * homog)
                    ? 1.0 : 0.0;
}

template <int W>
__global__ void __launch_bounds__(64 * W) k_cut_prep(KParams p) {
    extern __shared__ double prep_lds[];
    const int b = blockIdx.x;
    const int lane = threadIdx.x & 63, wv = W > 1 ? (int)(threadIdx.x >> 6) : 0;
    const int nls = p.tr.n_matched_ls[b];
    const int npt = p.tr.n_matched_pt[b];
    if (nls == 0) return;
    double (*chunk)[65] = reinterpret_cast<double (*)[65]>(prep_lds + (size_t)wv * 21 * 65);
    const DevCam& cam = p.cam;
    const double homog = p.cfg.homog_th;
    DevLines& L = p.prev.ls;
    const DevPoints& P = p.prev.pt;
    const size_t lb = (size_t)b * p.kl_cap, pbase = (size_t)b * p.kp_cap;
    const int32_t* mls = p.tr.matched_ls + (size_t)b * p.mls_cap;
    const int32_t* mpt = p.tr.matched_pt + (size_t)b * p.mpt_cap;
    double* rec_l = p.scr.cut_rec + LINE_SLOT(p, b, 0) * CUT_REC;
    double Dl[16];
    {
        double Tc[16], Tp[16], Ti[16];
#pragma unroll
        for (int i = 0; i < 16; ++i) { Tc[i] = p.curr.pose.Tfw[16 * b + i]; Tp[i] = p.prev.pose.Tfw[16 * b + i]; }
        mat4_inv(Tc, Ti);
        mat4_mul(Ti, Tp, Dl);
    }
    if (wv == 0 && lane < 16) p.scr.cut_dtinv[16 * b + lane] = Dl[lane];
    double s = 0.0;
    const int nl_ch = (nls + 63) >> 6, np_ch = (npt + 63) >> 6;
    auto chunk_cnt = [&](int c) {
        const bool lines = c < nl_ch;
        return min(64, (lines ? nls : npt) - (((lines ? c : c - nl_ch)) << 6));
    };
    for (int c0 = 0; c0 < nl_ch + np_ch; c0 += W) {
        const int c = c0 + wv;
        if (c < nl_ch + np_ch) {
            const bool lines = c < nl_ch;
            const int m = ((lines ? c : c - nl_ch) << 6) + lane;
            const int cnt = chunk_cnt(c);
            double info[21];
            double fd[CUT_FAST];
            if (lane < cnt) {
                if (lines) {
                    LineCutData d;
                    load_line(L, lb + mls[m], d);
                    poseInfoOnLine<false>(cam, homog, Dl, d, 0.0, 0.0, info);
#pragma unroll
                    for (int i = PD_ERR; i < CUT_FAST; ++i) fd[i] = 0.0;
                    cut_poly_data(Dl, d, homog, fd);
                    fd[PD_NEXT] = (double)mls[min(m + 1, nls - 1)];
                } else {
                    const size_t q = pbase + mpt[m];
                    double Pp[3] = {P.P[3 * q], P.P[3 * q + 1], P.P[3 * q + 2]};
                    double cur[3], uv[2];
                    se3_apply(Dl, Pp, cur);
                    projection(cam, cur, uv);
                    const double dx = uv[0] - P.pl_obs[2 * q], dy = uv[1] - P.pl_obs[2 * q + 1];
                    double J[6];
                    poseJac(cam, homog, cur, dx, dy, J);
#pragma unroll
                    for (int i = 0; i < 6; ++i)
#pragma unroll
                        for (int j = 0; j <= i; ++j) info[tri(i, j)] = J[i] * J[j];
                }
            }
            if (lines) {
                double* stg = &chunk[0][0];
                const int pl = lane >> 3, pp = lane & 7;
                double* rc = rec_l + (size_t)(c << 6) * CUT_REC;
#pragma unroll
                for (int sl = 0; sl < CUT_REC / 16; ++sl) {
                    if (lane < cnt) {
#pragma unroll
                        for (int k = 0; k < 16; ++k) {
                            const int x = 16 * sl + k;
                            stg[lane * 17 + k] = x < CUT_FAST ? fd[x] : (x < CUT_FAST + 21 ? info[x - CUT_FAST] : 0.0);
                        }
                    }
                    wave_lds_sync();
#pragma unroll
                    for (int g8 = 0; g8 < 8; ++g8) {
                        const int ln = 8 * g8 + pl;
                        if (ln < cnt)
                            reinterpret_cast<double2*>(rc + (size_t)ln * CUT_REC + 16 * sl)[pp] =
                                make_double2(stg[ln * 17 + 2 * pp], stg[ln * 17 + 2 * pp + 1]);
                    }
                    wave_lds_sync();
                }
            }
            if (lane < cnt) {
#pragma unroll
                for (int i = 0; i < 21; ++i) chunk[i][lane] = info[i];
            }
        }
        __syncthreads();
        if (wv == 0 && lane < 21) {
            const double (*all)[21][65] = reinterpret_cast<const double (*)[21][65]>(prep_lds);
            for (int k = 0; k < W && c0 + k < nl_ch + np_ch; ++k) {
                const int cnt = chunk_cnt(c0 + k);
                for (int e = 0; e < cnt; ++e) s = s + all[k][lane][e];
            }
        }
        __syncthreads();
    }
    if (wv == 0 && lane < 21) p.scr.cut_sum[CUT_SUM_REC * b + lane] = s;
}
constexpr size_t cut_prep_lds(int w) { return (size_t)w * 21 * 65 * sizeof(double); }

__device__ __forceinline__ float ceil_f32(double x) {
    if (!(x >= 0.0)) return __builtin_inff();
    float f = (float)x;
    if ((double)f < x) f = __uint_as_float(__float_as_uint(f) + 1u);
    return f;
}
template <bool SD>
__device__ __forceinline__ double ref_vprime_at(const DevCam& cam, double homog, const double* Dl, const double* P0,
                                                const double* P1, const double* C0, const double* C1, const double* Jl,
                                                double c) {
    double Pt[3];
#pragma unroll
    for (int k = 0; k < 3; ++k) Pt[k] = (1.0 - c) * P0[k] + c * P1[k];
    const double a = (1.0 - c) * (1.0 - c), qq = c * c;
    double cov[9];
#pragma unroll
    for (int i = 0; i < 9; ++i) cov[i] = a * C0[i] + qq * C1[i];
    const double v = endpointVar_t<double, SD>(cam, Dl, Jl, Pt, cov, 0.0);
    double cur[3];
    se3_apply(Dl, Pt, cur);
// ... 1443 lines not shown
            double tot[21];
            if (open) {
#pragma unroll
                for (int e = 0; e < 21; ++e) tot[e] = smat[g][e];
            } else {
                double S7[7], E7[7], info[21];
                const double* d = lnd[g];
                cut_endpoint(cam, homog, dti[g], d + 24, d, d + 3, d + 6, d + 15, t0, S7);
                cut_endpoint(cam, homog, dti[g], d + 24, d + 3, d, d + 15, d + 6, t1, E7);
                cut_assemble<false>(S7, E7, info);
#pragma unroll
                for (int e = 0; e < 21; ++e) {
                    ninf[g][21 * j + e] = info[e];
                    tot[e] = info[e] + smat[g][e];
                }
            }
            double A[36], w[6];
#pragma unroll
            for (int i = 0; i < 6; ++i)
#pragma unroll
                for (int k = 0; k <= i; ++k) {
                    A[i * 6 + k] = tot[tri(i, k)];
                    A[k * 6 + i] = tot[tri(i, k)];
                }
            int sw = 0;
            eig_sym<6, true>(A, w, &sw);
            v = w[0];
            if (!open || j == 0) {
                n_sweeps += sw;
                ++n_eval;
            }
        }
        wave_lds_sync();
        double top;
        const int best = group_first_max(v, valid, j, mc, top);
        if (live && open) {
            mc = v;
            open = 0;
#pragma unroll
            for (int kk = 0; kk < 3; ++kk) {
                const int e = j + 8 * kk;
                if (e < 21) smat[g][e] = ss[kk];
            }
        } else if (live) {
            ++n_steps;
            bool fin = true;
            if (best >= 0) {
#pragma unroll
                for (int kk = 0; kk < 3; ++kk) {
                    const int e = j + 8 * kk;
                    if (e < 21) ci[kk] = ninf[g][21 * best + e];
                }
                r0 = r0 + nb_step(best, 0, st);
                r1 = r1 + nb_step(best, 1, st);
                mc = top;
                fin = !(r0 + r1 <= 1.0);
            }
            if (fin) {
                if (j == 0) {
                    L.cut[2 * q_cur] = r0;
                    L.cut[2 * q_cur + 1] = r1;
                }
#pragma unroll
                for (int kk = 0; kk < 3; ++kk) se[kk] = ss[kk] + ci[kk];
                ++m;
                if (m < nls) open_line();
            }
        }
    }
    n_sweeps += __shfl_xor(n_sweeps, 1); n_sweeps += __shfl_xor(n_sweeps, 2); n_sweeps += __shfl_xor(n_sweeps, 4);
    n_eval += __shfl_xor(n_eval, 1); n_eval += __shfl_xor(n_eval, 2); n_eval += __shfl_xor(n_eval, 4);
    if (seq && j == 0) {
        step_rec(p.scr.bytes, b)[GFPL_STEP_CUT_STEPS] = n_steps;
        step_rec(p.scr.bytes, b)[GFPL_STEP_CUT_EXACT] = n_steps;
        step_rec(p.scr.bytes, b)[GFPL_STEP_CUT_UNBOUNDED] = 0;
        dbg_row(p.scr.dbg, b)[DBG_EIG_SWEEPS] = n_sweeps;
        dbg_row(p.scr.dbg, b)[DBG_EIG_EVALS] = n_eval;
    }
}

#ifndef GFPL_FIN_WAVES
#define GFPL_FIN_WAVES 4
#endif
__global__ void __launch_bounds__(64, GFPL_FIN_WAVES) k_cut_finish(KParams p) {
    const int b = blockIdx.x;
    const int nls = p.tr.n_matched_ls[b];
    if (nls == 0) return;
    const bool ends_only = p.cfg.cut_with_max_vol && (p.cfg.cut_proof == 1 || p.cfg.cut_proof == 3) &&
                           p.scr.cut_flag[b] == 0;
    const DevCam& cam = p.cam;
    DevLines& L = p.prev.ls;
    const size_t lb = (size_t)b * p.kl_cap;
    const int32_t* mls = p.tr.matched_ls + (size_t)b * p.mls_cap;
    double Dl[16];
#pragma unroll
    for (int i = 0; i < 16; ++i) Dl[i] = p.scr.cut_dtinv[16 * b + i];
    for (int m0 = 0; m0 < nls; m0 += 64) {
        const int m = m0 + (int)threadIdx.x;
        const bool live = m < nls;
        const size_t q = lb + (live ? mls[m] : 0);
        LineCutData d;
        double r0 = 0.0, r1 = 0.0;
        double info[36];
        if (live && ends_only) {
            load_line(L, q, d);
            r0 = L.cut[2 * q];
            r1 = L.cut[2 * q + 1];
        } else if (live) {
            load_line(L, q, d);
            r0 = L.cut[2 * q];
            r1 = L.cut[2 * q + 1];
            poseInfoOnLine<true>(cam, p.cfg.homog_th, Dl, d, r0, r1, info);
            double2* iv = reinterpret_cast<double2*>(L.invcov + 36 * q);
#pragma unroll
            for (int i = 0; i < 18; ++i) iv[i] = make_double2(info[2 * i], info[2 * i + 1]);
        }
        if (live && !(fabs(r0) < 0.0001 && fabs(r1) < 0.0001)) {
            double sP[3] = {d.sP[0], d.sP[1], d.sP[2]}, eP[3] = {d.eP[0], d.eP[1], d.eP[2]};
            if (fabs(r0) > 0.0001) {
                double s[3];
                for (int k = 0; k < 3; ++k) s[k] = (1 - r0) * sP[k] + r0 * eP[k];
                for (int k = 0; k < 3; ++k) { sP[k] = s[k]; L.sP[3 * q + k] = s[k]; }
                double uv[2];
                projection(cam, sP, uv);
                L.spl[2 * q] = uv[0]; L.spl[2 * q + 1] = uv[1];
                L.sdisp[q] = (cam.fx * cam.b) / sP[2];
            }
            if (fabs(r1) > 0.0001) {
                double e[3];
                for (int k = 0; k < 3; ++k) e[k] = (1 - r1) * eP[k] + r1 * sP[k];
                for (int k = 0; k < 3; ++k) { eP[k] = e[k]; L.eP[3 * q + k] = e[k]; }
                double uv[2];
                projection(cam, eP, uv);
                L.epl[2 * q] = uv[0]; L.epl[2 * q + 1] = uv[1];
                L.edisp[q] = (cam.fx * cam.b) / eP[2];
            }
        }
    }
}

__device__ __forceinline__ void vref_replay(const KParams& p, int b, int m) {
    const double* fd = p.scr.cut_rec + LINE_SLOT(p, b, m) * CUT_REC;
    double* out = p.scr.cut_vmax + LINE_SLOT(p, b, m) * CUT_VMAX;
    const uint8_t* path = p.scr.cut_path + LINE_SLOT(p, b, m) * CUT_PATH;
    const DevLines& L = p.prev.ls;
    const size_t q = (size_t)b * p.kl_cap + p.tr.matched_ls[LINE_SLOT(p, b, m)];
    const double* Dl = p.scr.cut_dtinv + 16 * (size_t)b;
    const double st = p.cfg.cut_step, rlo = p.cfg.cut_rng[0], rhi = p.cfg.cut_rng[1];
    double sP[3], eP[3], cS[9], cE[9], Jl[2], qs[5], qe[5];
#pragma unroll
    for (int k = 0; k < 3; ++k) { sP[k] = L.sP[3 * q + k]; eP[k] = L.eP[3 * q + k]; }
#pragma unroll
    for (int k = 0; k < 9; ++k) { cS[k] = L.covS[9 * q + k]; cE[k] = L.covE[9 * q + k]; }
    Jl[0] = L.le_obs[3 * q];
    Jl[1] = L.le_obs[3 * q + 1];
#pragma unroll
    for (int k = 0; k < 5; ++k) { qs[k] = fd[PD_VS + k]; qe[k] = fd[PD_VE + k]; }
    double r0 = 0.0, r1 = 0.0;
    bool done = false;
    long long ct0[4] = {-1, -1, -1, -1}, ct1[4] = {-1, -1, -1, -1};
    double cv0[4] = {0, 0, 0, 0}, cv1[4] = {0, 0, 0, 0};
    int slot0 = 0, slot1 = 0;
    double ivm[2] = {0.0, 0.0}, rim[2] = {0.0, 0.0};
    int marg = 0, nbad = 0, nev = 0;
    for (int k = 0; k < CUT_PATH && !done; ++k) {
        const int by = path[k];
        if (!(by & CUT_P_EXACT)) {
            ++marg;
            for (int w = 0; w < 6; ++w) {
                const int side = w >= 3 ? 1 : 0, o = w - 3 * side;
                const double rc = side ? r1 : r0;
                const double t = o == 0 ? rc + (-st) : (o == 2 ? rc + st : rc);
                if (!(t >= rlo && t <= rhi)) continue;
                const long long tb = __double_as_longlong(t);
                double vr = 0.0;
                bool hit = false;
#pragma unroll
                for (int z = 0; z < 4; ++z) {
                    const bool h = side ? ct1[z] == tb : ct0[z] == tb;
                    vr = h ? (side ? cv1[z] : cv0[z]) : vr;
                    hit = hit || h;
                }
                if (!hit) {
                    vr = side ? ref_vprime_at<true>(p.cam, p.cfg.homog_th, Dl, eP, sP, cE, cS, Jl, t)
                              : ref_vprime_at<true>(p.cam, p.cfg.homog_th, Dl, sP, eP, cS, cE, Jl, t);
                    ++nev;
#pragma unroll
                    for (int z = 0; z < 4; ++z) {
                        if (side && slot1 == z) { ct1[z] = tb; cv1[z] = vr; }
                        if (!side && slot0 == z) { ct0[z] = tb; cv0[z] = vr; }
                    }
                    if (side) slot1 = (slot1 + 1) & 3; else slot0 = (slot0 + 1) & 3;
                }
                const double* qc = side ? qe : qs;
                const double vo = __builtin_fma(t, __builtin_fma(t, __builtin_fma(t, __builtin_fma(t, qc[4], qc[3]), qc[2]),
                                                                 qc[1]), qc[0]);
                const double lo = fmin(vr, vo);
                const double rv = fabs(vo - vr) / vr;
                if (!(lo > 0.0 && rv < 0.01)) { ++nbad; continue; }
                const double iv = 1.01 / lo;
                ivm[side] = fmax(ivm[side], iv);
                rim[side] = fmax(rim[side], rv * iv);
            }
        }
        if (by & CUT_P_STAY) {
            done = true;
        } else {
            const int jj = by & 7;
            r0 = r0 + nb_step(jj, 0, st);
            r1 = r1 + nb_step(jj, 1, st);
            if (!(r0 + r1 <= 1.0)) done = true;
        }
    }
    if (!done || __double_as_longlong(r0) != __double_as_longlong(L.cut[2 * q]) ||
        __double_as_longlong(r1) != __double_as_longlong(L.cut[2 * q + 1]))
        nbad += 1 << 20;
    out[0] = ivm[0];
    out[1] = rim[0];
// ... 527 lines not shown
        PHASE_TICK(vk, 4);
        if (detail) {
            const int slot = atomicAdd(p.scr.cut_dtln, 1);
            if (slot < CUT_DTL * p.B) {
                double* e = p.scr.cut_dtl + (size_t)slot * CUT_DTL_REC;
#pragma unroll
                for (int i = 0; i < CUT_INFO; ++i) e[DTL_S + i] = fr[i][lane];
                e[DTL_K0] = K0; e[DTL_A1] = A1; e[DTL_B1] = B1; e[DTL_CS] = cs; e[DTL_CE] = ce; e[DTL_R0] = R0;
                e[DTL_RTS] = rts; e[DTL_RTE] = rte;
                e[DTL_OK] = line_ok ? 1.0 : 0.0;
                p.scr.cut_dtln[1 + slot] = b * p.mls_cap + m;
            } else {
                bad |= 1024;
            }
        }
        wave_lds_sync();
    }
    int mask = bad;
    int wl = lane;
#pragma unroll
    for (int o = 32; o > 0; o >>= 1) {
        mask |= __shfl_xor(mask, o);
        const double ow = __shfl_xor(worst, o);
        const int ol = __shfl_xor(wl, o);
        if (ow > worst || (ow == worst && ol < wl)) { worst = ow; wl = ol; }
    }
    tS = __shfl(tS, wl); tK = __shfl(tK, wl); tA = __shfl(tA, wl); tV = __shfl(tV, wl);
    bad = mask != 0 ? 1 : 0;
#pragma unroll
    for (int o = 32; o > 0; o >>= 1) {
        n_marg += __shfl_xor(n_marg, o);
        n_eval += __shfl_xor(n_eval, o);
        n_mline += __shfl_xor(n_mline, o);
        n_xchk += __shfl_xor(n_xchk, o);
        n_dline += __shfl_xor(n_dline, o);
    }
    if (lane == 0) {
        p.scr.cut_flag[b] = bad;
        step_rec(p.scr.bytes, b)[GFPL_STEP_PROOF_REDONE] = bad;
        step_rec(p.scr.bytes, b)[GFPL_STEP_PROOF_STEPS] = n_marg;
        step_rec(p.scr.bytes, b)[GFPL_STEP_PROOF_VREF] = n_eval;
        step_rec(p.scr.bytes, b)[GFPL_STEP_PROOF_LINES] = n_mline;
        dbg_row(p.scr.dbg, b)[DBG_VFY_MASK] = mask;
        dbg_row(p.scr.dbg, b)[DBG_VFY_WORST] = __double_as_longlong(worst);
        dbg_row(p.scr.dbg, b)[DBG_VFY_XCHK] = n_xchk;
        dbg_row(p.scr.dbg, b)[DBG_VFY_DLINES] = n_dline;
        dbg_row(p.scr.dbg, b)[DBG_VFY_TS] = __double_as_longlong(tS);
        dbg_row(p.scr.dbg, b)[DBG_VFY_TK] = __double_as_longlong(tK);
        dbg_row(p.scr.dbg, b)[DBG_VFY_TA] = __double_as_longlong(tA);
        dbg_row(p.scr.dbg, b)[DBG_VFY_TV] = __double_as_longlong(tV);
        if (VCLOCK) vk.store(dbg_row(p.scr.dbg, b));
    }
}

__global__ void __launch_bounds__(64) k_cut_verify_detail(KParams p) {
    const int n = min(p.scr.cut_dtln[0], CUT_DTL * p.B);
    for (int i = blockIdx.x * 64 + threadIdx.x; i < n; i += gridDim.x * 64) {
        const int e = p.scr.cut_dtln[1 + i];
        const int b = e / p.mls_cap, m = e % p.mls_cap;
        const double* pl = p.scr.cut_dtl + (size_t)i * CUT_DTL_REC;
        const size_t q = (size_t)b * p.kl_cap + p.tr.matched_ls[LINE_SLOT(p, b, m)];
        const double* fd = p.scr.cut_rec + LINE_SLOT(p, b, m) * CUT_REC;
        const uint8_t* path = p.scr.cut_path + LINE_SLOT(p, b, m) * CUT_PATH;
        double Dl[16];
#pragma unroll
        for (int k = 0; k < 16; ++k) Dl[k] = p.scr.cut_dtinv[16 * b + k];
        int nx = 0;
        const int bad = verify_line_detail(p, Dl, q, path, fd, p.prev.ls.cut[2 * q], p.prev.ls.cut[2 * q + 1], pl[DTL_K0],
                                           pl[DTL_A1], pl[DTL_B1], pl[DTL_CS], pl[DTL_CE], pl[DTL_R0], pl[DTL_RTS],
                                           pl[DTL_RTE], pl[DTL_OK] != 0.0, pl + DTL_S, 1, nx);
        if (bad) {
            atomicOr(&p.scr.cut_flag[b], 1);
            atomicOr(reinterpret_cast<unsigned long long*>(&step_rec(p.scr.bytes, b)[GFPL_STEP_PROOF_REDONE]), 1ull);
        }
        if (nx)
            atomicAdd(reinterpret_cast<unsigned long long*>(&dbg_row(p.scr.dbg, b)[DBG_VFY_XCHK]), (unsigned long long)nx);
    }
}

static int cut_wave_max_b() { return env_int("GFPL_CUT_WAVE_MAX_B", CUT_WAVE_MAX_B); }

static int cut_prep_w8_max_b() { return env_int("GFPL_CUT_PREP_W8_MAX_B", 256); }

hipError_t launch_line_cut(const KParams& p, hipStream_t s, const hipEvent_t* marks) {
    const int mode = p.cfg.cut_proof;
    const dim3 gsearch((p.B + CUT_G - 1) / CUT_G);
    if (p.B <= cut_prep_w8_max_b()) {
        static std::atomic<unsigned long long> attr{0};
        const hipError_t e = ensure_dyn_lds(reinterpret_cast<const void*>(k_cut_prep<8>), (int)cut_prep_lds(8), &attr);
        if (e != hipSuccess) return e;
        hipLaunchKernelGGL(k_cut_prep<8>, dim3(p.B), dim3(512), cut_prep_lds(8), s, p);
    } else {
        hipLaunchKernelGGL(k_cut_prep<1>, dim3(p.B), dim3(64), cut_prep_lds(1), s, p);
    }
    if (!p.cfg.cut_with_max_vol) {
        if (marks) (void)hipEventRecord(marks[0], s);
        hipLaunchKernelGGL(k_cut_search_eig, gsearch, dim3(64), 0, s, p);
        if (marks) (void)hipEventRecord(marks[1], s);
        hipLaunchKernelGGL(k_cut_finish, dim3(p.B), dim3(64), 0, s, p);
        return hipGetLastError();
    }
    if (mode == 2) {
        hipLaunchKernelGGL(k_cut_bounds, dim3((p.mls_cap + 63) / 64, p.B), dim3(64), 0, s, p);
        hipLaunchKernelGGL(k_cut_vtab, dim3(p.B), dim3(256), 0, s, p);
    }
    if (marks) (void)hipEventRecord(marks[0], s);
    if (mode == 2)
        hipLaunchKernelGGL(k_cut_search<true>, gsearch, dim3(64), 0, s, p);
    else if (p.B <= cut_wave_max_b())
        hipLaunchKernelGGL(k_cut_search_w, dim3(p.B), dim3(64), 0, s, p);
    else if (mode == 1 || mode == 3)
        hipLaunchKernelGGL(HIP_KERNEL_NAME(k_cut_search<false, true>), gsearch, dim3(64), 0, s, p);
    else
        hipLaunchKernelGGL(k_cut_search<false>, gsearch, dim3(64), 0, s, p);
    if (marks) (void)hipEventRecord(marks[1], s);
    if (mode == 1 || mode == 3) {
        if (hipMemsetAsync(p.scr.cut_offl, 0, sizeof(int32_t), s) != hipSuccess) return hipGetLastError();
        hipLaunchKernelGGL(k_cut_vref, dim3((p.mls_cap + 63) / 64, p.B), dim3(64), 0, s, p);
        hipLaunchKernelGGL(k_cut_vref_off, dim3(256), dim3(64), 0, s, p);
        hipLaunchKernelGGL(k_cut_ebound, dim3((p.mls_cap + 63) / 64, p.B), dim3(64), 0, s, p);
        if (hipMemsetAsync(p.scr.cut_dtln, 0, sizeof(int32_t), s) != hipSuccess) return hipGetLastError();
        hipLaunchKernelGGL(k_cut_verify, dim3(p.B), dim3(64), 0, s, p);
        hipLaunchKernelGGL(k_cut_verify_detail, dim3(256), dim3(64), 0, s, p);
        hipLaunchKernelGGL(k_cut_bounds, dim3((p.mls_cap + 63) / 64, p.B), dim3(64), 0, s, p);
        hipLaunchKernelGGL(k_cut_vtab, dim3(p.B), dim3(256), 0, s, p);
        hipLaunchKernelGGL(k_cut_search<true>, gsearch, dim3(64), 0, s, p);
    }
    hipLaunchKernelGGL(k_cut_finish, dim3(p.B), dim3(64), 0, s, p);
    return hipGetLastError();
}

}
```

### gf-pl-slam_amd/csrc/k_stereo.hip

```cpp
#include <type_traits>

#include "gfpl_kernels.hpp"
#include "gfpl_knn.hpp"
#include "gfpl_wave.hpp"

namespace gfpl {

template <typename K>
__device__ void bitonic_sort(K* a, int n) {
    for (int k = 2; k <= n; k <<= 1)
        for (int j = k >> 1; j > 0; j >>= 1) {
            for (int i = threadIdx.x; i < n; i += blockDim.x) {
                int ixj = i ^ j;
                if (ixj > i) {
                    bool up = ((i & k) == 0);
                    K x = a[i], y = a[ixj];
                    if ((x > y) == up) { a[i] = y; a[ixj] = x; }
                }
            }
            __syncthreads();
        }
}

template <typename K>
// ... 654 lines not shown
        p.curr.pose.time_stamp[b] = p.in.time_stamp[b];
        p.scr.n_subpix[b] = misc[2];
    }
    DIAG_STAMP(GFPL_SP_CLOCK, threadIdx.x == 0, dbg_row(p.scr.dbg, blockIdx.x), 5);
}

#ifndef GFPL_SL_PRIO
#define GFPL_SL_PRIO 1
#endif
#if GFPL_SL_PRIO
#define SL_PRIO(k) __builtin_amdgcn_s_setprio(k)
#else
#define SL_PRIO(k) do { } while (0)
#endif
struct LineOut {
    double spl[2], epl[2], sdisp, edisp, sP[3], eP[3], le[3], angle;
    int level;
};

__device__ __forceinline__ int eig_gate_bound(const double* C, double th) {
    double M = 0.0, G = -__builtin_inf(), D = -__builtin_inf();
    bool fin = true;
#pragma unroll
    for (int i = 0; i < 9; ++i) { fin = fin && (C[i] - C[i] == 0.0); M = fmax(M, fabs(C[i])); }
    if (!fin) return -1;
#pragma unroll
    for (int i = 0; i < 3; ++i) {
        const double d = C[4 * i];
        const double r = (d + fabs(C[3 * i + (i + 1) % 3])) + fabs(C[3 * i + (i + 2) % 3]);
        G = fmax(G, r);
        D = fmax(D, d);
    }
    if (D >= th) return 0;
    if (G + 4e-9 * M < th) return 1;
    return -1;
}

__device__ bool triangulate(const KParams& p, const gfpl_keyline& a, const gfpl_keyline& c, bool initial,
                            LineOut* L) {
    const DevCam& cam = p.cam;
    double sp_l[3] = {a.sx, a.sy, 1.0}, ep_l[3] = {a.ex, a.ey, 1.0};
    double le_l[3] = {sp_l[1] * ep_l[2] - sp_l[2] * ep_l[1], sp_l[2] * ep_l[0] - sp_l[0] * ep_l[2],
                      sp_l[0] * ep_l[1] - sp_l[1] * ep_l[0]};
    double nrm = sqrt(le_l[0] * le_l[0] + le_l[1] * le_l[1]);
    le_l[0] = le_l[0] / nrm; le_l[1] = le_l[1] / nrm; le_l[2] = le_l[2] / nrm;
    double sp_r[3] = {c.sx, c.sy, 1.0}, ep_r[3] = {c.ex, c.ey, 1.0};
    double le_r[3] = {sp_r[1] * ep_r[2] - sp_r[2] * ep_r[1], sp_r[2] * ep_r[0] - sp_r[0] * ep_r[2],
                      sp_r[0] * ep_r[1] - sp_r[1] * ep_r[0]};
    double overlap = overlapStereo(sp_l[1], ep_l[1], sp_r[1], ep_r[1]);
    double spx = (-(le_r[2] + le_r[1] * (double)a.sy)) / le_r[0];
    double epx = (-(le_r[2] + le_r[1] * (double)a.ey)) / le_r[0];
    double disp_s = (double)a.sx - spx;
    double disp_e = (double)a.ex - epx;
    double horiz = initial ? (double)fabsf((float)le_r[0]) : (double)fabsf((float)le_l[0]);
    if (!(disp_s >= p.cfg.min_disp && disp_e >= p.cfg.min_disp && horiz > p.cfg.line_horiz_th &&
          overlap > p.cfg.stereo_overlap_th))
        return false;
    if (!initial) {
        double cS[9], cE[9];
        endpointCov(cam, sp_l[0], sp_l[1], disp_s, cS);
        endpointCov(cam, ep_l[0], ep_l[1], disp_e, cE);
        const double th = p.cfg.line_cov_th;
        const int gS = eig_gate_bound(cS, th), gE = eig_gate_bound(cE, th);
        if (gS == 0 || gE == 0) return false;
        if (!(gS == 1 && gE == 1)) {
            double wS[3], wE[3];
            eig_sym<3>(cS, wS);
            eig_sym<3>(cE, wE);
            double max_eig = std_max(wS[2], wE[2]);
            if (!(max_eig < th)) return false;
        }
    }
    L->spl[0] = sp_l[0]; L->spl[1] = sp_l[1];
    L->epl[0] = ep_l[0]; L->epl[1] = ep_l[1];
    L->sdisp = disp_s; L->edisp = disp_e;
    backProjection(cam, sp_l[0], sp_l[1], disp_s, L->sP);
    backProjection(cam, ep_l[0], ep_l[1], disp_e, L->eP);
    L->le[0] = le_l[0]; L->le[1] = le_l[1]; L->le[2] = le_l[2];
    L->angle = (double)a.angle;
    L->level = a.octave;
    return true;
}

__device__ void line_uncertainty(const KParams& p, const double* spl, const double* epl, double sdisp,
                                 double edisp, const double* le, double* covS, double* covE) {
    double sdisp_std, edisp_std;
    if (fabs(le[0]) > 0.15) {
        sdisp_std = p.cfg.ratio_disp_std * sdisp;
        edisp_std = p.cfg.ratio_disp_std * edisp;
    } else {
        sdisp_std = p.cfg.ratio_disp_std_hor * sdisp;
        edisp_std = p.cfg.ratio_disp_std_hor * edisp;
    }
    covMat2D_3D(p.cam, spl[0], spl[1], 1.0, sdisp, sdisp_std, covS);
    covMat2D_3D(p.cam, epl[0], epl[1], 1.0, edisp, edisp_std, covE);
}

__device__ void write_line(const KParams& p, DevLines& C, size_t q, const LineOut& L, int idx, const uint8_t* desc) {
    C.spl[2 * q] = L.spl[0]; C.spl[2 * q + 1] = L.spl[1];
    C.epl[2 * q] = L.epl[0]; C.epl[2 * q + 1] = L.epl[1];
    C.sdisp[q] = L.sdisp; C.edisp[q] = L.edisp;
    for (int k = 0; k < 3; ++k) { C.sP[3 * q + k] = L.sP[k]; C.eP[3 * q + k] = L.eP[k]; C.le[3 * q + k] = L.le[k]; }
    C.angle[q] = L.angle;
    C.level[q] = L.level;
    C.sigma2[q] = p.cam.sigma2_ln[clamp_level(L.level, GFPL_MAX_LEVELS)];
    C.idx[q] = idx;
    C.inlier[q] = 1;
    C.cut[2 * q] = 0.0; C.cut[2 * q + 1] = 0.0;
    const uint4* s = reinterpret_cast<const uint4*>(desc);
    uint4* d = reinterpret_cast<uint4*>(C.desc + q * 32);
    d[0] = s[0]; d[1] = s[1];
}

template <int CELL, bool INITIAL, int BLOCK>
__global__ void __launch_bounds__(BLOCK, GFPL_SL_WAVES) k_stereo_lines(KParams p) {
    extern __shared__ __align__(16) unsigned char smem[];
    const int b = blockIdx.x;
    const int cap = p.kl_cap;
    uint32_t* lut = (uint32_t*)smem;
    uint32_t* tb = lut + knn_lut_dwords(CELL);
    int* lr_i = (int*)(tb + cap * 8);
    int* lr_d0 = lr_i + cap;
    int* lr_d1 = lr_d0 + cap;
    int* rl_i = lr_d1 + cap;
    int* hist = rl_i + cap;
    int* misc = hist + 260;
    const int tid = threadIdx.x;
    const int NL = min(p.in.n_kl_l[b], cap), NR = min(p.in.n_kl_r[b], cap);
    DevLines& C = p.curr.ls;
    if (NL < 2 || NR < 2) {
        if (tid == 0) C.n[b] = 0;
        return;
    }
    const uint8_t* DLg = p.in.ldesc_l + (size_t)b * cap * 32;
    const uint8_t* DRg = p.in.ldesc_r + (size_t)b * cap * 32;
    DIAG_STAMP(GFPL_SL_CLOCK, threadIdx.x == 0 && !INITIAL, dbg_row(p.scr.dbg, blockIdx.x), 0);
    SL_PRIO(3);
    knn_stage_views<CELL>(tb, cap, DRg, NR);
    for (int i = tid; i < 260; i += blockDim.x) hist[i] = 0;
    for (int j = tid; j < NR; j += blockDim.x) rl_i[j] = -1;
    knn_lut_fill<CELL>(lut);
    __syncthreads();
    DIAG_STAMP(GFPL_SL_CLOCK, threadIdx.x == 0 && !INITIAL, dbg_row(p.scr.dbg, blockIdx.x), 1);
    knn2_mfma<CELL>(tb, cap, NR, DLg, NL, (uint32_t*)lr_i, (uint32_t*)lr_d1, (uint32_t*)rl_i);
    __syncthreads();
    DIAG_STAMP(GFPL_SL_CLOCK, threadIdx.x == 0 && !INITIAL, dbg_row(p.scr.dbg, blockIdx.x), 2);
    SL_PRIO(1);
    for (int i = tid; i < NL; i += blockDim.x) {
        const uint32_t k0 = (uint32_t)lr_i[i], k1 = (uint32_t)lr_d1[i];
        const int d0 = (int)(k0 >> 16), d1 = (int)(k1 >> 16);
        lr_i[i] = (int)(k0 & 0xFFFFu); lr_d0[i] = d0; lr_d1[i] = d1;
        atomicAdd(&hist[d1 - d0], 1);
    }
    for (int j = tid; j < NR; j += blockDim.x) rl_i[j] = (int)((uint32_t)rl_i[j] & KNN_IDX_MASK);
    __syncthreads();
    if (tid < 64) {
        const int v = wave_hist_rank(hist, NL / 2, 257);
        if (tid == 0) {
            double th = (1.4826 * (double)(float)v) * p.cfg.desc_th_l;
            reinterpret_cast<double*>(misc + 8)[0] = th;
        }
    }
    __syncthreads();
    const double nn12_dist_th = reinterpret_cast<double*>(misc + 8)[0];
    DIAG_STAMP(GFPL_SL_CLOCK, threadIdx.x == 0 && !INITIAL, dbg_row(p.scr.dbg, blockIdx.x), 3);
    const int n_matches = min(NL, NR);
    const gfpl_keyline* KL = p.in.kl_l + (size_t)b * cap;
    const gfpl_keyline* KR = p.in.kl_r + (size_t)b * cap;
    const size_t base = (size_t)b * cap;
    int off = 0;
    for (int c0 = 0; c0 < n_matches; c0 += BLOCK) {
        const int i = c0 + tid;
        int flag = 0;
        LineOut L;
        if (i < n_matches) {
            const int lr_tdx = lr_i[i];
            const int rl_tdx = rl_i[lr_tdx];
            const double dist_12 = (double)((float)lr_d1[i] - (float)lr_d0[i]);
            if (i == rl_tdx && dist_12 > nn12_dist_th)
                flag = triangulate(p, KL[i], KR[lr_tdx], INITIAL, &L) ? 1 : 0;
// ... 20 lines not shown
    }
    const int32_t* lr = p.scr.knn + (size_t)b * 2 * cap * 3;
    const int32_t* rl = lr + (size_t)cap * 3;
    const gfpl_keypoint* KL = p.in.kp_l + (size_t)b * cap;
    const gfpl_keypoint* KR = p.in.kp_r + (size_t)b * cap;
    const uint8_t* DL = p.in.pdesc_l + (size_t)b * cap * 32;
    const size_t base = (size_t)b * cap;
    int off = 0;
    for (int c0 = 0; c0 < N; c0 += 512) {
        const int i = c0 + tid;
        int flag = 0;
        double disp_ = 0.0;
        if (i < N) {
            const int t = lr[3 * i];
            const int rl_tdx = rl[3 * t];
            const double dist_12 = (double)((float)lr[3 * i + 1] / (float)lr[3 * i + 2]);
            if (i == rl_tdx && dist_12 <= p.cfg.max_ratio_12_p) {
                const gfpl_keypoint kl = KL[i], kr = KR[t];
                if ((double)fabsf(kl.y - kr.y) <= p.cfg.max_dist_epip) {
                    disp_ = (double)(kl.x - kr.x);
                    if (disp_ >= p.cfg.min_disp) flag = 1;
                }
            }
        }
        int tot;
        const int pos = off + block_exclusive_scan<512>(flag, misc, &tot);
        if (flag) {
            const gfpl_keypoint kl = KL[i];
            const size_t q = base + pos;
            double P[3];
            const double plx = kl.x, ply = kl.y;
            backProjection(p.cam, plx, ply, disp_, P);
            C.pl[2 * q] = plx; C.pl[2 * q + 1] = ply;
            C.disp[q] = disp_;
            C.P[3 * q] = P[0]; C.P[3 * q + 1] = P[1]; C.P[3 * q + 2] = P[2];
            C.sigma2[q] = p.cam.sigma2_pt[clamp_level(kl.octave, p.cam.n_levels)];
            C.idx[q] = pos;
            C.level[q] = kl.octave;
            C.inlier[q] = 1;
            const uint4* s = reinterpret_cast<const uint4*>(DL + (size_t)i * 32);
            uint4* d = reinterpret_cast<uint4*>(C.desc + q * 32);
            d[0] = s[0]; d[1] = s[1];
        }
        off += tot;
    }
    if (tid == 0) {
        C.n[b] = off;
        p.curr.pose.time_stamp[b] = p.in.time_stamp[b];
    }
}

__global__ void k_init_pose(KParams p) {
    const int b = blockIdx.x * blockDim.x + threadIdx.x;
    if (b >= p.B) return;
    DevPose& P = p.curr.pose;
    for (int i = 0; i < 16; ++i) { P.Tfw[16 * b + i] = (i % 5 == 0) ? 1.0 : 0.0; P.DT[16 * b + i] = (i % 5 == 0) ? 1.0 : 0.0; }
    for (int i = 0; i < 36; ++i) { P.Tfw_cov[36 * b + i] = (i % 7 == 0) ? 1.0 : 0.0; P.DT_cov[36 * b + i] = 0.0; }
    for (int i = 0; i < 6; ++i) P.DT_cov_eig[6 * b + i] = 0.0;
    P.err_norm[b] = 0.0;
    p.tr.num_frame_loss[b] = 0;
    p.tr.n_matched_pt[b] = 0;
    p.tr.n_matched_ls[b] = 0;
    p.tr.n_inliers[b] = 0; p.tr.n_inliers_pt[b] = 0; p.tr.n_inliers_ls[b] = 0;
    for (int i = 0; i < 16; ++i) p.tr.kf_T[16 * b + i] = (i % 5 == 0) ? 1.0 : 0.0;
    for (int i = 0; i < 36; ++i) p.tr.kf_cov[36 * b + i] = 0.0;
    p.tr.kf_prev_iskf[b] = 1;
    p.tr.kf_nsince[b] = 0;
    p.tr.kf_entropy0[b] = 0.0;
    p.tr.kf_ratio[b] = 0.0;
    p.tr.kf_flag[b] = 0;
}

__global__ void __launch_bounds__(256) k_line_uncertainty(KParams p) {
    __shared__ double cs[256 * 9], ce[256 * 9];
    const int b = blockIdx.y;
    const int i0 = blockIdx.x * blockDim.x;
    const int i = i0 + threadIdx.x;
    DevLines& L = p.prev.ls;
    const int n = L.n[b];
    if (i0 >= n) return;
    if (i < n) {
        const size_t q = (size_t)b * p.kl_cap + i;
        double spl[2] = {L.spl[2 * q], L.spl[2 * q + 1]}, epl[2] = {L.epl[2 * q], L.epl[2 * q + 1]};
        double le[3] = {L.le[3 * q], L.le[3 * q + 1], L.le[3 * q + 2]};
        double cS[9], cE[9];
        line_uncertainty(p, spl, epl, L.sdisp[q], L.edisp[q], le, cS, cE);
#pragma unroll
        for (int k = 0; k < 9; ++k) { cs[9 * threadIdx.x + k] = cS[k]; ce[9 * threadIdx.x + k] = cE[k]; }
    }
    __syncthreads();
    const int m = 9 * min(256, n - i0);
    double* dS = L.covS + 9 * ((size_t)b * p.kl_cap + i0);
    double* dE = L.covE + 9 * ((size_t)b * p.kl_cap + i0);
    for (int k = threadIdx.x; k < m; k += 256) { dS[k] = cs[k]; dE[k] = ce[k]; }
}

__global__ void k_step_bytes(KParams p) {
    const int b = blockIdx.x * blockDim.x + threadIdx.x;
    if (b >= p.B) return;
    const int64_t No = (int64_t)p.in.n_kp_l[b] + p.in.n_kp_r[b];
    const int64_t Nk = (int64_t)p.in.n_kl_l[b] + p.in.n_kl_r[b];
    const int64_t Mo = p.scr.n_subpix[b];
    const int64_t Sp = p.prev.pt.n[b], Sl = p.prev.ls.n[b];
    const int64_t Sp2 = p.curr.pt.n[b], Sl2 = p.curr.ls.n[b];
    const int64_t Mp = p.tr.n_matched_pt[b], Ml = p.tr.n_matched_ls[b];
    int64_t st[6];
    st[0] = 44 * No + (121 + 231) * Mo + 97 * Sp2;
    st[1] = 56 * Nk + 193 * Sl2;
    st[2] = 216 * Sl + 60 * Sp + 48 * Sp2 + 25 * Mp + 256;
    st[3] = 36 * Sl + 32 * Sl2 + 153 * Ml;
    st[4] = 608 * Ml + 44 * Mp;
    st[5] = 54 * Mp + 86 * Ml + 1504;
    int64_t tot = 0;
    int64_t* rec = step_rec(p.scr.bytes, b);
    for (int i = 0; i < 6; ++i) { rec[GFPL_STEP_B_STEREO_POINTS + i] = st[i]; tot += st[i]; }
    rec[GFPL_STEP_B_TOTAL] = tot;
    rec[GFPL_STEP_B_CUT_SEARCH] = (p.cfg.use_line_conf_cut && Ml > 0) ? 396 * Ml + 272 : 0;
    rec[GFPL_STEP_N_O] = No; rec[GFPL_STEP_N_K] = Nk; rec[GFPL_STEP_M_O] = Mo; rec[GFPL_STEP_S_P] = Sp2;
    rec[GFPL_STEP_S_L] = Sl2; rec[GFPL_STEP_M_P] = Mp; rec[GFPL_STEP_M_L] = Ml;
    rec[GFPL_STEP_N_INLIERS] = p.tr.n_inliers[b];
    if (!(p.cfg.use_line_conf_cut && Ml > 0)) rec[GFPL_STEP_CUT_STEPS] = rec[GFPL_STEP_CUT_EXACT] = 0;
    rec[GFPL_STEP_INLIERS_POSE] = rec[GFPL_STEP_N_INLIERS];
    if (!(p.cfg.use_line_conf_cut && Ml > 0)) rec[GFPL_STEP_CUT_UNBOUNDED] = 0;
    if (!(p.cfg.use_line_conf_cut && p.cfg.cut_with_max_vol && (p.cfg.cut_proof == 1 || p.cfg.cut_proof == 3)))
        rec[GFPL_STEP_PROOF_REDONE] = rec[GFPL_STEP_PROOF_STEPS] = rec[GFPL_STEP_PROOF_VREF] =
            rec[GFPL_STEP_PROOF_LINES] = 0;
    p.tr.kf_nsince[b] = p.tr.kf_nsince[b] + 1;
}

static inline int next_pow2(int v) { int p = 1; while (p < v) p <<= 1; return p; }

#ifndef SP_WIDE_MAX_B
#define SP_WIDE_MAX_B 256
#endif
int sp_wide_max_b() { return env_int("GFPL_SP_WIDE_MAX_B", SP_WIDE_MAX_B); }

hipError_t launch_stereo_points(const KParams& p, hipStream_t s) {
    const int KP2 = next_pow2(p.kp_cap);
    auto lds_of = [&](bool seg, int waves) {
        return (size_t)StereoPointsLds(nullptr, KP2, p.cam.height, p.cam.n_levels, seg, waves).bytes;
    };
    const size_t lds_seg = lds_of(true, 8), lds_seg_w = lds_of(true, 16);
    if (p.B <= sp_wide_max_b() && p.kp_cap <= 2048 && lds_seg_w <= 64 * 1024) {
        hipLaunchKernelGGL((k_stereo_points<1024, true>), dim3(p.B), dim3(1024), lds_seg_w, s, p, KP2);
        return hipGetLastError();
    }
    if (p.kp_cap > 2048) {
        static std::atomic<unsigned long long> attr{0};
        const hipError_t e = ensure_dyn_lds(reinterpret_cast<const void*>(k_stereo_points<1024, false>), DYN_LDS_CEILING, &attr);
        if (e != hipSuccess) return e;
        hipLaunchKernelGGL((k_stereo_points<1024, false>), dim3(p.B), dim3(1024), lds_of(false, 16), s, p, KP2);
    }
    else if (lds_seg <= 54 * 1024 && p.kp_cap <= 2048)
        hipLaunchKernelGGL((k_stereo_points<512, true>), dim3(p.B), dim3(512), lds_seg, s, p, KP2);
    else
        hipLaunchKernelGGL((k_stereo_points<512, false>), dim3(p.B), dim3(512), lds_of(false, 8), s, p, KP2);
    return hipGetLastError();
}

template <int CELL, bool INITIAL, int BLOCK>
static hipError_t launch_stereo_lines_as(const KParams& p, hipStream_t s) {
    if (BLOCK == 1024) {
        static std::atomic<unsigned long long> attr{0};
        const hipError_t e = ensure_dyn_lds(reinterpret_cast<const void*>(k_stereo_lines<CELL, INITIAL, BLOCK>),
                                            DYN_LDS_CEILING, &attr);
        if (e != hipSuccess) return e;
    }
    hipLaunchKernelGGL((k_stereo_lines<CELL, INITIAL, BLOCK>), dim3(p.B), dim3(BLOCK),
                       StereoLinesLds(nullptr, p.kl_cap, CELL).bytes, s, p);
// ... 34 lines not shown
```

### gf-pl-slam_amd/gfpl/__init__.py

```python
from __future__ import annotations

import ctypes as C
import enum
import json
import os
from typing import Optional

import numpy as np

PKG_DIR = os.path.dirname(os.path.dirname(os.path.abspath(__file__)))
LIB_DIR = os.path.join(PKG_DIR, "lib")
REPO_DIR = os.path.dirname(PKG_DIR)

DESC = 32
MAX_LEVELS = 8
MAX_MATCHED_PT = 2048
MAX_MATCHED_LS = 1024
PREV, CURR = 0, 1
HAMMING, HAMMING2 = 1, 2

ERRORS = {0: "ok", -1: "invalid argument", -2: "HIP runtime error", -3: "no HIP device",
          -4: "knn-2 needs at least 2 train descriptors", -5: "capacity exceeded",
          -6: "call order violated", -7: "unsupported config", -8: "device memory allocation failed"}

# ... 484 lines not shown
            "gfpl_config_default": ([P], C.c_int),
            "gfpl_camera_init": ([P, C.c_int, C.c_int, C.c_double, C.c_double, C.c_double,
                                  C.c_double, C.c_double, P], C.c_int),
            "gfpl_create": ([C.c_int, P, C.POINTER(P)], C.c_int),
            "gfpl_create_async": ([C.c_int, C.POINTER(P)], C.c_int),
            "gfpl_get_stream": ([P], C.c_void_p),
            "gfpl_event_create": ([P, C.POINTER(P)], C.c_int),
            "gfpl_event_destroy": ([P], C.c_int),
            "gfpl_event_record": ([P, P], C.c_int),
            "gfpl_event_wait": ([P, P], C.c_int),
            "gfpl_event_synchronize": ([P], C.c_int),
            "gfpl_event_record_count": ([P, P], C.c_int),
            "gfpl_orb_extract_async": ([P, P, C.c_int, P, P, P, P, P, P, C.c_int64], C.c_int),
            "gfpl_orb_status": ([P], C.c_int),
            "gfpl_lsd_detect_async": ([P, P, C.c_int, P, P, P], C.c_int),
            "gfpl_lsd_status": ([P], C.c_int),
            "gfpl_lbd_compute_async": ([P, P, C.c_int, P, P, P], C.c_int),
            "gfpl_lbd_status": ([P], C.c_int),
            "gfpl_destroy": ([P], C.c_int),
            "gfpl_set_camera": ([P, P], C.c_int),
            "gfpl_set_config": ([P, P], C.c_int),
            "gfpl_get_camera": ([P, P], C.c_int),
            "gfpl_get_config": ([P, P], C.c_int),
            "gfpl_synchronize": ([P], C.c_int),
            "gfpl_copy_to_host": ([P, P, P, C.c_size_t], C.c_int),
            "gfpl_seqbatch_create": ([P, C.c_int, C.c_int, C.c_int, C.POINTER(P)], C.c_int),
            "gfpl_seqbatch_destroy": ([P], C.c_int),
            "gfpl_seqbatch_bytes": ([P], C.c_int64),
            "gfpl_initialize": ([P, P], C.c_int),
            "gfpl_insert_stereo_pair": ([P, P], C.c_int),
            "gfpl_optimize_pose": ([P], C.c_int),
            "gfpl_optimize_pose_ini": ([P, P], C.c_int),
            "gfpl_update_frame": ([P], C.c_int),
            "gfpl_frame_step": ([P, P], C.c_int),
            "gfpl_upload_frames": ([P, P, P], C.c_int),
            "gfpl_upload_frames_async": ([P, P, C.c_int, C.c_int, P], C.c_int),
            "gfpl_upload_wait": ([P, C.c_int64], C.c_int),
            "gfpl_upload_frames_l0_async": ([P, P, C.c_int, C.c_int, C.c_int64, P], C.c_int),
            "gfpl_staged_frames": ([P, C.c_int, P], C.c_int),
            "gfpl_stereo_points": ([P, P], C.c_int),
            "gfpl_stereo_lines": ([P, P], C.c_int),
            "gfpl_line_uncertainty": ([P], C.c_int),
            "gfpl_cross_points": ([P], C.c_int),
            "gfpl_cross_lines": ([P], C.c_int),
            "gfpl_line_cut": ([P], C.c_int),
            "gfpl_knn2_hamming": ([P, P, C.c_int, P, C.c_int, C.c_int, P, P], C.c_int),
            "gfpl_kf_common_matches": ([P, P, P, P, P, P, P], C.c_int),
            "gfpl_kf_local_map_matches": ([P, P, P, C.c_double, C.c_double, P, P, P, P], C.c_int),
            "gfpl_default_loop_params": ([P], None),
            "gfpl_default_fuse_params": ([P], None),
            "gfpl_map_fuse_search": ([P, P, P, P, P, P, P, P, P, P, P], C.c_int),
            "gfpl_map_fuse_debug_ms": ([P, C.c_int, P], C.c_int),
            "gfpl_kf_loop_closure": ([P, P, P, C.c_int, P, C.c_int, C.c_int, P, P, P, P, P], C.c_int),
            "gfpl_vocab_create": ([P, P, P], C.c_int),
            "gfpl_vocab_destroy": ([P], C.c_int),
            "gfpl_vocab_check": ([P], C.c_int),
            "gfpl_bow_transform": ([P, P, C.c_int, P, P, C.c_int, P, P, P], C.c_int),
            "gfpl_bow_score": ([P, P, P, C.c_int, P], C.c_int),
            "gfpl_kf_bow_stats": ([P, C.c_int, P, P, C.c_int, P], C.c_int),
            "gfpl_bowdb_create": ([P, P, P, C.c_int, C.c_int, C.c_int, C.c_int, P], C.c_int),
            "gfpl_bowdb_destroy": ([P], C.c_int),
            "gfpl_bowdb_insert": ([P, C.c_int, P, P, P], C.c_int),
            "gfpl_bowdb_erase": ([P, C.c_int], C.c_int),
            "gfpl_bowdb_vector": ([P, C.c_int, C.c_int, P, P, P], C.c_int),
            "gfpl_default_lc_search_params": ([P], None),
            "gfpl_kf_loop_candidates": ([P, P, P, C.c_int, P, P, P], C.c_int),
            "gfpl_read_frame": ([P, C.c_int, C.c_int, P], C.c_int),
            "gfpl_write_frame": ([P, C.c_int, C.c_int, P], C.c_int),
            "gfpl_read_track": ([P, C.c_int, P], C.c_int),
            "gfpl_read_last_track": ([P, C.c_int, P], C.c_int),
            "gfpl_need_new_kf": ([P, P], C.c_int),
            "gfpl_curr_frame_is_kf": ([P, P], C.c_int),
            "gfpl_read_kf_state": ([P, C.c_int, P], C.c_int),
            "gfpl_write_track": ([P, C.c_int, P], C.c_int),
            "gfpl_set_timing": ([P, C.c_int], C.c_int),
            "gfpl_get_stage_times": ([P, P], C.c_int),
            "gfpl_get_kernel_times": ([P, P], C.c_int),
            "gfpl_last_step_kernel_bytes": ([P, P], C.c_int),
            "gfpl_last_step_bytes": ([P, P], C.c_int),
            "gfpl_last_step_stage_bytes": ([P, P], C.c_int),
            "gfpl_last_step_counts": ([P, P], C.c_int),
            "gfpl_last_step_track_counts": ([P, P], C.c_int),
            "gfpl_last_step_cut_proof": ([P, P], C.c_int),
            "gfpl_debug_cut_records": ([P, C.c_int, P, C.c_int], C.c_int),
            "gfpl_debug_step_records": ([P, P], C.c_int),
            "gfpl_debug_clocks": ([P, P], C.c_int),
            "gfpl_lsd_create": ([P, P, C.c_int, C.c_int, C.c_int, C.c_int, C.c_int, C.POINTER(P)], C.c_int),
            "gfpl_lsd_destroy": ([P], C.c_int),
            "gfpl_lsd_detect": ([P, P, C.c_int, P, P, P], C.c_int),
            "gfpl_lsd_sort_desc": ([P, P, C.c_int], C.c_int),
            "gfpl_strerror": ([C.c_int], C.c_char_p),
            "gfpl_orb_create": ([P, C.c_int, C.c_int, P, C.c_int, C.c_int, C.POINTER(P)], C.c_int),
            "gfpl_orb_destroy": ([P], C.c_int),
            "gfpl_orb_pyramid_bytes": ([P, P], C.c_int),
            "gfpl_orb_extract": ([P, P, C.c_int, P, P, P, P, P, P, C.c_int64], C.c_int),
            "gfpl_lbd_create": ([P, C.c_int, C.c_int, C.c_int, C.c_int, C.POINTER(P)], C.c_int),
            "gfpl_lbd_destroy": ([P], C.c_int),
            "gfpl_lbd_compute": ([P, P, C.c_int, P, P, P], C.c_int),
            "gfpl_lbd_gradients": ([P, P, P], C.c_int),
            "gfpl_detector_params_default": ([P, P, P], C.c_int),
            "gfpl_detector_create": ([P, P, C.c_int, C.c_int, C.c_int, C.c_int, C.POINTER(P)], C.c_int),
            "gfpl_detector_destroy": ([P], C.c_int),
            "gfpl_detect_stereo_async": ([P, P, P, C.c_int, P, P], C.c_int),
            "gfpl_detect_stereo_host": ([P, P, P, C.c_int, P, P], C.c_int),
            "gfpl_detect_stereo": ([P, P, P, C.c_int, P, C.c_int, P], C.c_int),
            "gfpl_detector_status": ([P], C.c_int),
            "gfpl_detector_discard": ([P, P], C.c_int),
            "gfpl_read_detections": ([P, P, C.c_int, P], C.c_int),
            "gfpl_rectify_maps_host": ([P, C.c_int, C.c_int, P, P], C.c_int),
            "gfpl_rectifier_create": ([P, P, P, C.c_int, C.c_int, C.POINTER(P)], C.c_int),
            "gfpl_rectifier_destroy": ([P], C.c_int),
            "gfpl_rectifier_read_maps": ([P, C.c_int, P, P], C.c_int),
            "gfpl_rectify": ([P, C.c_int, P, C.c_int, P], C.c_int),
            "gfpl_rectify_async": ([P, C.c_int, P, C.c_int, P], C.c_int),
            "gfpl_rectify_stereo_async": ([P, P, P, C.c_int, P, P], C.c_int),
            "gfpl_rectify_host": ([P, C.c_int, P, C.c_int, P], C.c_int),
            "gfpl_detector_set_rectifier": ([P, P], C.c_int),
            "gfpl_default_lba_params": ([P], None),
            "gfpl_lba_check": ([P], C.c_int),
            "gfpl_lba_workspace": ([P, P, P], C.c_int),
            "gfpl_lba_create": ([P, P, C.c_int, C.POINTER(P)], C.c_int),
            "gfpl_lba_destroy": ([P], C.c_int),
            "gfpl_lba_solve": ([P, P, C.c_int, P, P], C.c_int),
            "gfpl_lba_debug_system": ([P, C.c_int, C.c_int, P, P, P, P, P, P, P], C.c_int),
            "gfpl_lmstore_create": ([P, C.c_int, C.c_int, C.c_int, C.POINTER(P)], C.c_int),
            "gfpl_lmstore_destroy": ([P], C.c_int),
            "gfpl_lmstore_bytes": ([P], C.c_int64),
            "gfpl_lm_ops_check": ([P, C.c_int, P, C.c_int, C.c_int, P, C.c_int], C.c_int),
            "gfpl_lmstore_apply": ([P, P, C.c_int, P, P, C.c_int], C.c_int),
            "gfpl_lm_fuse_check": ([P, C.c_int, P, C.c_int, C.c_int, P, C.c_int, P], C.c_int),
            "gfpl_lmstore_fuse": ([P, P, C.c_int, P, P, C.c_int], C.c_int),
            "gfpl_lmstore_gather": ([P, P, C.c_int, P, P], C.c_int),
            "gfpl_lmstore_read": ([P, C.c_int, P, P, P, P], C.c_int),
            "gfpl_lmstore_debug_ms": ([P, P], C.c_int),
            "gfpl_default_kfmap_params": ([P], None),
            "gfpl_kfmap_bytes": ([P], C.c_int64),
            "gfpl_kfmap_create": ([P, P, C.POINTER(P)], C.c_int),
            "gfpl_kfmap_destroy": ([P], C.c_int),
            "gfpl_kfmap_counts": ([P, P, P, P], C.c_int),
            "gfpl_kfmap_add_keyframe": ([P, C.c_int, C.c_int, P], C.c_int),
            "gfpl_kfmap_observe_pairs": ([P, C.c_int, C.c_int, C.c_int, P, C.c_int, P, P, P], C.c_int),
            "gfpl_kfmap_observe_local": ([P, C.c_int, C.c_int, P, C.c_int, P, C.c_int, P, C.c_int, P], C.c_int),
            "gfpl_kfmap_form_local_map": ([P, P], C.c_int),
            "gfpl_kfmap_select": ([P, C.c_int, C.c_int, C.c_int, P, P], C.c_int),
            "gfpl_kfmap_unmatched": ([P, C.c_int, C.c_int, P, P], C.c_int),
            "gfpl_kfmap_local_keyframes": ([P, P, P], C.c_int),
            "gfpl_kfmap_remove_bad": ([P, P, P, P, P, P], C.c_int),
            "gfpl_kfmap_set_inlier": ([P, C.c_int, P, C.c_int, C.c_int], C.c_int),
            "gfpl_kfmap_erase_keyframe": ([P, C.c_int], C.c_int),
            "gfpl_kfmap_read_keyframe": ([P, C.c_int, P, P, P], C.c_int),
            "gfpl_kfmap_write_keyframe_idx": ([P, C.c_int, C.c_int, C.c_int, C.c_int, P], C.c_int),
            "gfpl_kfmap_read_landmarks": ([P, C.c_int, C.c_int, C.c_int, P, P, P, P, P, P], C.c_int),
            "gfpl_kfmap_write_landmarks": ([P, C.c_int, C.c_int, C.c_int, P, P, P, P, P, P], C.c_int),
            "gfpl_kfmap_export_graph": ([P, P, P, P, P, P, P, P, P], C.c_int),
            "gfpl_kfmap_debug_ms": ([P, P], C.c_int),
            "gfpl_mapgeo_bytes": ([P], C.c_int64),
            "gfpl_mapgeo_create": ([P, P, C.POINTER(P)], C.c_int),
            "gfpl_mapgeo_destroy": ([P], C.c_int),
            "gfpl_mapgeo_set_keyframe": ([P, C.c_int, P, P], C.c_int),
            "gfpl_mapgeo_read_keyframe": ([P, C.c_int, P, P], C.c_int),
            "gfpl_mapgeo_arrays": ([P, P, P, P, P], C.c_int),
            "gfpl_mapgeo_observe_pairs": ([P, C.c_int, C.c_int, C.c_int, P, P, P, P, C.c_int, C.c_int], C.c_int),
            "gfpl_mapgeo_observe_local": ([P, C.c_int, C.c_int, P, P, C.c_int, P, C.c_int, P], C.c_int),
            "gfpl_mapgeo_free": ([P, C.c_int, P, C.c_int], C.c_int),
            "gfpl_mapgeo_read_landmarks": ([P, C.c_int, C.c_int, C.c_int, P, P, P, P], C.c_int),
            "gfpl_mapgeo_write_landmarks": ([P, C.c_int, C.c_int, C.c_int, P, P, P, P], C.c_int),
# ... 1431 lines not shown
    def upload_async(self, host: Frames, s0: int, slot: int, l0_stride: int = 0) -> int:
        t = C.c_int64()
        if l0_stride > 0:
            check(self.L.gfpl_upload_frames_l0_async(self.h, C.byref(host), s0, slot, l0_stride, C.byref(t)),
                  "upload_frames_l0_async")
        else:
            check(self.L.gfpl_upload_frames_async(self.h, C.byref(host), s0, slot, C.byref(t)), "upload_frames_async")
        return t.value

    def upload_wait(self, ticket: int):
        check(self.L.gfpl_upload_wait(self.h, ticket), "upload_wait")

    def staged_frames(self, slot: int) -> Frames:
        dev = Frames()
        check(self.L.gfpl_staged_frames(self.h, slot, C.byref(dev)), "staged_frames")
        return dev

    def read_frame(self, which: int, seq: int) -> FrameHost:
        fh = FrameHost(self.kp_cap, self.kl_cap)
        check(self.L.gfpl_read_frame(self.h, which, seq, fh.ptr()), "read_frame")
        return fh

    def write_frame(self, which: int, seq: int, fh: FrameHost):
        check(self.L.gfpl_write_frame(self.h, which, seq, fh.ptr()), "write_frame")

    def read_track(self, seq: int) -> dict:
        t = TrackHost()
        check(self.L.gfpl_read_track(self.h, seq, C.byref(t)), "read_track")
        return t.as_dict()

    def read_last_track(self, seq: int) -> dict:
        t = TrackHost()
        check(self.L.gfpl_read_last_track(self.h, seq, C.byref(t)), "read_last_track")
        return t.as_dict()

    def needNewKF(self) -> np.ndarray:
        flags = np.zeros(self.B, np.int32)
        check(self.L.gfpl_need_new_kf(self.h, flags.ctypes.data), "need_new_kf")
        return flags.astype(bool)

    def currFrameIsKF(self, mask=None):
        if mask is None:
            check(self.L.gfpl_curr_frame_is_kf(self.h, None), "curr_frame_is_kf")
            return
        m = np.ascontiguousarray(np.broadcast_to(np.asarray(mask), (self.B,)), dtype=np.int32)
        check(self.L.gfpl_curr_frame_is_kf(self.h, m.ctypes.data), "curr_frame_is_kf")

    def read_kf_state(self, seq: int) -> dict:
        st = KFState()
        check(self.L.gfpl_read_kf_state(self.h, seq, C.byref(st)), "read_kf_state")
        return st.as_dict()

    def write_track(self, seq: int, tr: TrackHost):
        check(self.L.gfpl_write_track(self.h, seq, C.byref(tr)), "write_track")

    def last_step_bytes(self) -> int:
        v = C.c_int64()
        check(self.L.gfpl_last_step_bytes(self.h, C.byref(v)), "last_step_bytes")
        return v.value

    def last_step_stage_bytes(self) -> np.ndarray:
        v = np.zeros(7, np.int64)
        check(self.L.gfpl_last_step_stage_bytes(self.h, v.ctypes.data), "last_step_stage_bytes")
        return v

    STEP_COUNTS = ["N_o", "N_k", "M_o", "S_p", "S_l", "M_p", "M_l", "n_inliers"]

    def last_step_counts(self) -> dict:
        v = np.zeros(8, np.int64)
        check(self.L.gfpl_last_step_counts(self.h, v.ctypes.data), "last_step_counts")
        return {n: float(x) / self.B for n, x in zip(self.STEP_COUNTS, v)}

    def last_step_track_counts(self) -> dict:
        v = np.zeros(4, np.int64)
        check(self.L.gfpl_last_step_track_counts(self.h, v.ctypes.data), "last_step_track_counts")
        return {"steps": int(v[0]), "exact_steps": int(v[1]), "inliers_after_pose": int(v[2]),
                "lines_unbounded": int(v[3])}

    def last_step_cut_proof(self) -> dict:
        v = np.zeros(4, np.int64)
        check(self.L.gfpl_last_step_cut_proof(self.h, v.ctypes.data), "last_step_cut_proof")
        return {"redone": int(v[0]), "steps_proven": int(v[1]), "vref_evals": int(v[2]), "lines": int(v[3])}

    def debug_cut_records(self, b: int, n_lines: int) -> np.ndarray:
        out = np.zeros((n_lines, 80), np.float64)
        check(self.L.gfpl_debug_cut_records(self.h, b, out.ctypes.data, n_lines), "debug_cut_records")
        return out

    def debug_step_records(self) -> np.ndarray:
        out = np.zeros((self.B, STEP_REC), np.int64)
        check(self.L.gfpl_debug_step_records(self.h, out.ctypes.data), "debug_step_records")
        return out

    def debug_clocks(self) -> np.ndarray:
        out = np.zeros((self.B, 8), np.int64)
        check(self.L.gfpl_debug_clocks(self.h, out.ctypes.data), "debug_clocks")
        return out

    def last_step_kernel_bytes(self) -> np.ndarray:
        v = np.zeros(4, np.int64)
        check(self.L.gfpl_last_step_kernel_bytes(self.h, v.ctypes.data), "last_step_kernel_bytes")
        return v

    def nbytes(self) -> int:
        return int(self.L.gfpl_seqbatch_bytes(self.h))

    def close(self):
        if getattr(self, "h", None):
            self.L.gfpl_seqbatch_destroy(self.h)
            self.h = None

    def __del__(self):
        try:
            self.close()
        except Exception:
            pass


def track_from_dict(d: dict) -> TrackHost:
    t = TrackHost()
    t.n_matched_pt = len(d["matched_pt"])
    t.n_matched_ls = len(d["matched_ls"])
    for i, v in enumerate(d["matched_pt"]):
        t.matched_pt[i] = int(v)
    for i, v in enumerate(d["matched_ls"]):
        t.matched_ls[i] = int(v)
    t.n_inliers, t.n_inliers_pt, t.n_inliers_ls = d["n_inliers"], d["n_inliers_pt"], d["n_inliers_ls"]
    t.num_frame_loss = d["num_frame_loss"]
    return t


class ORBextractor:

    def __init__(self, nfeatures: int, scaleFactor: float, nlevels: int, iniThFAST: int, minThFAST: int,
                 width: int, height: int, max_images: int = 1, kp_cap: Optional[int] = None,
                 ctx: Optional[Context] = None, device: int = 0):
        self.L = hiplib()
        self.prm = OrbParams(nfeatures, scaleFactor, nlevels, iniThFAST, minThFAST)
        self.width, self.height, self.max_images = width, height, max_images
        self.kp_cap = kp_cap or nfeatures + 64 * nlevels + 64
        self._own = None
        if ctx is None:
            h = C.c_void_p()
            check(self.L.gfpl_create(device, None, C.byref(h)), "gfpl_create")
            self._own = h
            ch = h
        else:
            ch = ctx.h
        self._ctx = ctx
        o = C.c_void_p()
        check(self.L.gfpl_orb_create(ch, width, height, C.byref(self.prm), max_images, self.kp_cap, C.byref(o)),
              "orb_create")
        self.h = o
        b = C.c_int64()
        check(self.L.gfpl_orb_pyramid_bytes(o, C.byref(b)), "orb_pyramid_bytes")
        self.pyramid_bytes = b.value
        sc = [1.0]
        for _ in range(1, nlevels):
            sc.append(float(np.float32(sc[-1]) * np.float32(scaleFactor)))
        self.mvScaleFactor = np.array(sc, np.float32)
        self.mvLevelSigma2 = self.mvScaleFactor * self.mvScaleFactor
        self.mvInvScaleFactor = np.float32(1.0) / self.mvScaleFactor
        self.mvInvLevelSigma2 = np.float32(1.0) / self.mvLevelSigma2
        self.mvImagePyramid = []

    def GetLevels(self) -> int: return self.prm.nlevels
# ... 500 lines not shown
```

### include/gfpl.h

```cpp
#ifndef GFPL_H
#define GFPL_H

#include <stddef.h>
#include <stdint.h>

#ifdef __cplusplus
extern "C" {
#endif

#define GFPL_ABI_VERSION 6

#define GFPL_DESC_BYTES 32
#define GFPL_MAX_LEVELS 8
#define GFPL_MAX_IMAGE_DIM 2047
#define GFPL_MAX_MATCHED_PT 2048
#define GFPL_MAX_MATCHED_LS 1024
#define GFPL_PYR_TAIL 64

#define GFPL_OK                   0
#define GFPL_E_INVALID          (-1)
#define GFPL_E_HIP              (-2)
#define GFPL_E_NO_DEVICE        (-3)
#define GFPL_E_TOO_FEW_TRAIN    (-4)
#define GFPL_E_CAPACITY         (-5)
// ... 570 lines not shown
int  gfpl_mapgeo_read_landmarks(gfpl_mapgeo* g, int kind, int id0, int n, double* lm3d, int32_t* n_obs, double* obs, double* sigma);
int  gfpl_mapgeo_write_landmarks(gfpl_mapgeo* g, int kind, int id0, int n, const double* lm3d, const int32_t* n_obs,
                                 const double* obs, const double* sigma);
typedef struct gfpl_mapgeo_lists {
    int32_t *pt_obs_lm, *pt_obs_kf;
    int32_t *ls_obs_lm, *ls_obs_kf;
    int32_t cap_pt_obs, cap_ls_obs;
} gfpl_mapgeo_lists;
int  gfpl_mapgeo_assemble(gfpl_mapgeo* g, const gfpl_kfmap* kfmap, int which, gfpl_lba_problem* problem,
                          const gfpl_mapgeo_lists* lists);
int  gfpl_mapgeo_assembled_ids(gfpl_mapgeo* g, const int32_t** kf_list, const int32_t** fix_list, const int32_t** pt_list,
                               const int32_t** ls_list);
int  gfpl_mapgeo_read_assembled(gfpl_mapgeo* g, const gfpl_lba_problem* host, int32_t* kf_list, int32_t* fix_list,
                                int32_t* pt_list, int32_t* ls_list);
int  gfpl_mapgeo_lba(gfpl_mapgeo* g, const gfpl_kfmap* kfmap, gfpl_lba* lba, const gfpl_lba_params* prm,
                     gfpl_lba_result* result, gfpl_lba_counts* counts);
int  gfpl_mapgeo_debug_ms(gfpl_mapgeo* g, float* ms);

#define GFPL_PGO_COV 0
#define GFPL_PGO_ESS 1
typedef struct gfpl_pgo gfpl_pgo;
typedef struct gfpl_pgo_graph_params {
    int32_t min_lm_ess_graph, min_lm_cov_graph, variant, max_iters, max_rejects, pad;
    double  lambda_init;
} gfpl_pgo_graph_params;
void gfpl_default_pgo_params(gfpl_pgo_graph_params* prm);
typedef struct gfpl_pgo_counts { int32_t n_kf, n_lc, n_vert, n_free, n_edge, env_blocks, n_pt, n_ls; } gfpl_pgo_counts;
typedef struct gfpl_pgo_problem {
    int32_t        n_kf, n_lc;
    int32_t        n_pt, n_ls;
    const uint8_t* alive;
    const int32_t* full_graph;
    const int32_t* lc;
    const double*  lc_pose;
    double*        T_kf;
    double*        x_kf;
    double*        pt;
    double*        ls;
    double*        pt_dir;
    double*        ls_dir;
    const int32_t* pt_kf_start;
    const int32_t* pt_kf_idx;
    const int32_t* ls_kf_start;
    const int32_t* ls_kf_idx;
    const int32_t* pt_dir_off;
    const int32_t* ls_dir_off;
    const uint8_t* pt_freed;
    const uint8_t* ls_freed;
} gfpl_pgo_problem;
#define GFPL_PGO_STOP_ITERS  0
#define GFPL_PGO_STOP_STEP   1
#define GFPL_PGO_STOP_DCHI2  2
#define GFPL_PGO_STOP_REJECT 3
#define GFPL_PGO_STOP_NOFREE 4
#define GFPL_PGO_SINGULAR    1
typedef struct gfpl_pgo_result {
    int32_t iters, stop, status, rejects;
    int32_t n_vert, n_free, n_edge, kf_curr;
    double  lambda, chi2_0, chi2;
} gfpl_pgo_result;
int  gfpl_pgo_check(const gfpl_pgo_problem* p, const gfpl_pgo_graph_params* prm, gfpl_pgo_counts* counts);
int  gfpl_pgo_workspace(const gfpl_pgo_counts* n, int64_t* hbm_bytes, int32_t* lds_bytes);
int  gfpl_pgo_create(gfpl_ctx* ctx, const gfpl_pgo_counts* caps, int max_problems, gfpl_pgo** out);
int  gfpl_pgo_destroy(gfpl_pgo* pgo);
int  gfpl_pgo_solve(gfpl_pgo* pgo, const gfpl_pgo_problem* problems, int n, const gfpl_pgo_graph_params* prm,
                    gfpl_pgo_result* results);
int  gfpl_pgo_debug_system(gfpl_pgo* pgo, int i, double* chi2, double* b, double* diag, double* env,
                           int32_t* env_first, int32_t* vert, int32_t* edge, double* Z, double* X0);
int  gfpl_pgo_debug_ms(gfpl_pgo* pgo, float* ms_solve, float* ms_correct);

int  gfpl_read_frame(gfpl_seqbatch* sb, int which, int seq, gfpl_frame_host* out);
int  gfpl_write_frame(gfpl_seqbatch* sb, int which, int seq, const gfpl_frame_host* in);
int  gfpl_read_track(gfpl_seqbatch* sb, int seq, gfpl_track_host* out);
int  gfpl_write_track(gfpl_seqbatch* sb, int seq, const gfpl_track_host* in);
int  gfpl_read_last_track(gfpl_seqbatch* sb, int seq, gfpl_track_host* out);

int  gfpl_set_timing(gfpl_ctx* ctx, int enable);
int  gfpl_get_stage_times(gfpl_ctx* ctx, float* ms7);
int  gfpl_last_step_bytes(gfpl_seqbatch* sb, int64_t* bytes);
int  gfpl_last_step_stage_bytes(gfpl_seqbatch* sb, int64_t* bytes7);
int  gfpl_last_step_counts(gfpl_seqbatch* sb, int64_t* counts8);
int  gfpl_last_step_track_counts(gfpl_seqbatch* sb, int64_t* counts4);
int  gfpl_last_step_cut_proof(gfpl_seqbatch* sb, int64_t* counts4);
int  gfpl_debug_cut_records(gfpl_seqbatch* sb, int b, double* out, int n_lines);
enum {
    GFPL_STEP_B_STEREO_POINTS = 0,
    GFPL_STEP_B_STEREO_LINES = 1,
    GFPL_STEP_B_CROSS_POINTS = 2,
    GFPL_STEP_B_CROSS_LINES = 3,
    GFPL_STEP_B_LINE_CUT = 4,
    GFPL_STEP_B_POSE = 5,
    GFPL_STEP_B_TOTAL = 6,
    GFPL_STEP_B_CUT_SEARCH = 7,
    GFPL_STEP_N_O = 8,
    GFPL_STEP_N_K = 9,
    GFPL_STEP_M_O = 10,
    GFPL_STEP_S_P = 11,
    GFPL_STEP_S_L = 12,
    GFPL_STEP_M_P = 13,
    GFPL_STEP_M_L = 14,
    GFPL_STEP_N_INLIERS = 15,
    GFPL_STEP_CUT_STEPS = 16,
    GFPL_STEP_CUT_EXACT = 17,
    GFPL_STEP_INLIERS_POSE = 18,
    GFPL_STEP_CUT_UNBOUNDED = 19,
    GFPL_STEP_PROOF_REDONE = 20,
    GFPL_STEP_PROOF_STEPS = 21,
    GFPL_STEP_PROOF_VREF = 22,
    GFPL_STEP_PROOF_LINES = 23,
    GFPL_STEP_REC = 24
};
int  gfpl_debug_step_records(gfpl_seqbatch* sb, int64_t* out);
int  gfpl_debug_clocks(gfpl_seqbatch* sb, int64_t* out);
int  gfpl_get_kernel_times(gfpl_ctx* ctx, float* ms4);
int  gfpl_last_step_kernel_bytes(gfpl_seqbatch* sb, int64_t* bytes4);

const char* gfpl_strerror(int code);

#ifdef __cplusplus
}
#endif
#endif
```

Baseline: 810,200.

## Recompute line covariances on the fly in cut kernels when freshly formed

```diff
diff --git a/gf-pl-slam_amd/csrc/gfpl_abi.hip b/gf-pl-slam_amd/csrc/gfpl_abi.hip
--- a/gf-pl-slam_amd/csrc/gfpl_abi.hip
+++ b/gf-pl-slam_amd/csrc/gfpl_abi.hip
@@ -59,6 +59,9 @@
     int32_t* last_n_ls = nullptr;
     PyrBuild* pyrb = nullptr;
     int last_cut_mode = -1;
+    bool cov_fresh = false;
+    double cov_key[6] = {0, 0, 0, 0, 0, 0};
+    bool last_cut_cov = false;
 };
 
 struct gfpl_event {
@@ -184,6 +187,22 @@
     return d;
 }
 
+void cov_key(const gfpl_ctx* c, double* k) {
+    k[0] = c->cam.fx; k[1] = c->cam.cx; k[2] = c->cam.cy; k[3] = c->cam.b;
+    k[4] = c->cfg.ratio_disp_std; k[5] = c->cfg.ratio_disp_std_hor;
+}
+void cov_mark(gfpl_seqbatch* sb) {
+    cov_key(sb->ctx, sb->cov_key);
+    sb->cov_fresh = true;
+}
+bool cov_take(gfpl_seqbatch* sb) {
+    double k[6];
+    cov_key(sb->ctx, k);
+    const bool ok = sb->cov_fresh && std::memcmp(k, sb->cov_key, sizeof k) == 0;
+    sb->cov_fresh = false;
+    return ok;
+}
+
 KParams params(gfpl_seqbatch* sb, const gfpl_frames* in) {
     KParams p;
     std::memset(&p, 0, sizeof p);
@@ -489,6 +508,7 @@
     if (slot == -2) return GFPL_E_HIP;
     KParams p = params(sb, in);
     p.curr = sb->slot[sb->prev_slot];
+    sb->cov_fresh = false;
     HIPCHK(launch_init(p, sb->ctx->stream));
     sb->initialized = true;
     sb->has_curr = false;
@@ -522,7 +542,9 @@
 int gfpl_line_uncertainty(gfpl_seqbatch* sb) {
     if (!sb) return GFPL_E_INVALID;
     if (!sb->initialized) return GFPL_E_STATE;
+    sb->cov_fresh = false;
     HIPCHK(launch_line_uncertainty(params(sb, nullptr), sb->ctx->stream));
+    cov_mark(sb);
     return GFPL_OK;
 }
 
@@ -544,7 +566,8 @@
     if (!sb) return GFPL_E_INVALID;
     if (!sb->initialized || !sb->has_curr) return GFPL_E_STATE;
     sb->last_cut_mode = cut_mode(sb->ctx->cfg);
-    HIPCHK(launch_line_cut(params(sb, nullptr), sb->ctx->stream, nullptr));
+    const bool fresh = sb->last_cut_cov = cov_take(sb);
+    HIPCHK(launch_line_cut(params(sb, nullptr), sb->ctx->stream, nullptr, fresh));
     return GFPL_OK;
 }
 
@@ -557,19 +580,25 @@
     const int slot = in_acquire(sb, in);
     if (slot == -2) return GFPL_E_HIP;
     KParams p = params(sb, in);
+    sb->cov_fresh = false;
     tmark(c, 0);
     HIPCHK(launch_stereo_points(p, c->stream));
     tmark(c, 1);
     HIPCHK(launch_stereo_lines(p, c->stream));
     tmark(c, 2);
-    if (c->cfg.use_line_conf_cut) HIPCHK(launch_line_uncertainty(p, c->stream));
+    if (c->cfg.use_line_conf_cut) {
+        HIPCHK(launch_line_uncertainty(p, c->stream));
+        cov_mark(sb);
+    }
     HIPCHK(launch_cross_points(p, c->stream));
     tmark(c, 3);
     HIPCHK(launch_cross_lines(p, c->stream));
     tmark(c, 4);
     sb->last_cut_mode = c->cfg.use_line_conf_cut ? cut_mode(c->cfg) : -1;
-    if (c->cfg.use_line_conf_cut)
-        HIPCHK(launch_line_cut(p, c->stream, c->timing ? &c->ev[7] : nullptr));
+    if (c->cfg.use_line_conf_cut) {
+        const bool fresh = sb->last_cut_cov = cov_take(sb);
+        HIPCHK(launch_line_cut(p, c->stream, c->timing ? &c->ev[7] : nullptr, fresh));
+    }
     HIPCHK(launch_step_bytes(p, c->stream));
     tmark(c, 5);
     sb->has_curr = true;
@@ -783,6 +812,7 @@
     HIPCHK(hipMemsetAsync(sb->tr.n_matched_pt, 0, sizeof(int32_t) * sb->B, sb->ctx->stream));
     HIPCHK(hipMemsetAsync(sb->tr.n_matched_ls, 0, sizeof(int32_t) * sb->B, sb->ctx->stream));
     sb->prev_slot = 1 - sb->prev_slot;
+    sb->cov_fresh = false;
     sb->has_curr = false;
     return GFPL_OK;
 }
@@ -1336,6 +1366,7 @@
 int gfpl_write_frame(gfpl_seqbatch* sb, int which, int seq, const gfpl_frame_host* o) {
     if (!sb || !o || seq < 0 || seq >= sb->B || (which != GFPL_PREV && which != GFPL_CURR)) return GFPL_E_INVALID;
     if (o->n_pt < 0 || o->n_pt > sb->kp_cap || o->n_ls < 0 || o->n_ls > sb->kl_cap) return GFPL_E_CAPACITY;
+    sb->cov_fresh = false;
     hipStream_t s = sb->ctx->stream;
     const DevFrame& f = sb->slot[which == GFPL_PREV ? sb->prev_slot : 1 - sb->prev_slot];
     XFER(h2d, f.pt.n + seq, &o->n_pt, 1);
@@ -1361,6 +1392,7 @@
     if (!sb || !o || seq < 0 || seq >= sb->B) return GFPL_E_INVALID;
     if (o->n_matched_pt < 0 || o->n_matched_pt > sb->mpt_cap || o->n_matched_ls < 0 || o->n_matched_ls > sb->mls_cap)
         return GFPL_E_CAPACITY;
+    sb->cov_fresh = false;
     for (int i = 0; i < o->n_matched_pt; ++i)
         if (o->matched_pt[i] < 0 || o->matched_pt[i] >= sb->kp_cap) return GFPL_E_INVALID;
     for (int i = 0; i < o->n_matched_ls; ++i)
@@ -1461,6 +1493,11 @@
                          sb && (sb->last_cut_mode == 1 || sb->last_cut_mode == 3));
 }
 
+int gfpl_last_cut_formed_cov(gfpl_seqbatch* sb) {
+    if (!sb) return GFPL_E_INVALID;
+    return sb->last_cut_cov ? 1 : 0;
+}
+
 int gfpl_debug_cut_records(gfpl_seqbatch* sb, int b, double* out, int n_lines) {
     if (!sb || !out || b < 0 || b >= sb->B || n_lines < 0 || n_lines > sb->mls_cap) return GFPL_E_INVALID;
     if (hipSetDevice(sb->ctx->device) != hipSuccess) return GFPL_E_HIP;
diff --git a/gf-pl-slam_amd/csrc/gfpl_device.hpp b/gf-pl-slam_amd/csrc/gfpl_device.hpp
--- a/gf-pl-slam_amd/csrc/gfpl_device.hpp
+++ b/gf-pl-slam_amd/csrc/gfpl_device.hpp
@@ -881,6 +881,20 @@
             cov[i * 3 + j] = (JC[i * 3 + 0] * J[j * 3 + 0] + JC[i * 3 + 1] * J[j * 3 + 1]) + JC[i * 3 + 2] * J[j * 3 + 2];
 }
 
+GFPL_DEV void line_uncertainty(const DevCam& cam, const gfpl_config& cfg, const double* spl, const double* epl,
+                               double sdisp, double edisp, double le0, double* covS, double* covE) {
+    double sdisp_std, edisp_std;
+    if (fabs(le0) > 0.15) {
+        sdisp_std = cfg.ratio_disp_std * sdisp;
+        edisp_std = cfg.ratio_disp_std * edisp;
+    } else {
+        sdisp_std = cfg.ratio_disp_std_hor * sdisp;
+        edisp_std = cfg.ratio_disp_std_hor * edisp;
+    }
+    covMat2D_3D(cam, spl[0], spl[1], 1.0, sdisp, sdisp_std, covS);
+    covMat2D_3D(cam, epl[0], epl[1], 1.0, edisp, edisp_std, covE);
+}
+
 GFPL_DEV double std_min(double a, double b) { return (b < a) ? b : a; }
 GFPL_DEV double std_max(double a, double b) { return (a < b) ? b : a; }
 GFPL_DEV double overlapStereo(double spl_obs, double epl_obs, double spl_proj, double epl_proj) {
diff --git a/gf-pl-slam_amd/csrc/gfpl_kernels.hpp b/gf-pl-slam_amd/csrc/gfpl_kernels.hpp
--- a/gf-pl-slam_amd/csrc/gfpl_kernels.hpp
+++ b/gf-pl-slam_amd/csrc/gfpl_kernels.hpp
@@ -45,7 +45,7 @@
                               hipStream_t s);
 hipError_t launch_cross_points(const KParams& p, hipStream_t s);
 hipError_t launch_cross_lines(const KParams& p, hipStream_t s);
-hipError_t launch_line_cut(const KParams& p, hipStream_t s, const hipEvent_t* marks );
+hipError_t launch_line_cut(const KParams& p, hipStream_t s, const hipEvent_t* marks , bool cov_fresh);
 hipError_t launch_pose(const KParams& p, hipStream_t s, hipEvent_t mark );
 hipError_t launch_step_bytes(const KParams& p, hipStream_t s);
 hipError_t launch_need_kf(const KParams& p, hipStream_t s);
diff --git a/gf-pl-slam_amd/csrc/k_cut.hip b/gf-pl-slam_amd/csrc/k_cut.hip
--- a/gf-pl-slam_amd/csrc/k_cut.hip
+++ b/gf-pl-slam_amd/csrc/k_cut.hip
@@ -129,6 +129,59 @@
     d.Jl[1] = L.le_obs[3 * q + 1];
 }
 
+struct LineCovSrc {
+    double spl[2], epl[2], sdisp, edisp, le0;
+};
+__device__ __forceinline__ void load_cov_src(const DevLines& L, size_t q, LineCovSrc& c) {
+    c.spl[0] = L.spl[2 * q]; c.spl[1] = L.spl[2 * q + 1];
+    c.epl[0] = L.epl[2 * q]; c.epl[1] = L.epl[2 * q + 1];
+    c.sdisp = L.sdisp[q]; c.edisp = L.edisp[q];
+    c.le0 = L.le[3 * q];
+}
+__device__ __forceinline__ void form_cov(const DevCam& cam, const gfpl_config& cfg, const LineCovSrc& c, double* covS,
+                                         double* covE) {
+    line_uncertainty(cam, cfg, c.spl, c.epl, c.sdisp, c.edisp, c.le0, covS, covE);
+}
+__device__ __forceinline__ void load_line_ends(const DevLines& L, size_t q, LineCutData& d) {
+#pragma unroll
+    for (int k = 0; k < 3; ++k) { d.sP[k] = L.sP[3 * q + k]; d.eP[k] = L.eP[3 * q + k]; }
+    d.Jl[0] = L.le_obs[3 * q];
+    d.Jl[1] = L.le_obs[3 * q + 1];
+}
+__device__ __forceinline__ void load_line_cov(const DevCam& cam, const gfpl_config& cfg, const DevLines& L, size_t q,
+                                              LineCutData& d) {
+    LineCovSrc c;
+    load_cov_src(L, q, c);
+    form_cov(cam, cfg, c, d.covS, d.covE);
+    load_line_ends(L, q, d);
+}
+__device__ __forceinline__ void poseInfoOnLine_cov(const DevCam& cam, const gfpl_config& cfg, double homog,
+                                                   const double* DT_inv, const LineCutData& L, const DevLines& Ls,
+                                                   size_t q, double c0, double c1, double* info) {
+    double S7[7], E7[7];
+    {
+        LineCovSrc c;
+        double cS[9], cE[9];
+        load_cov_src(Ls, q, c);
+        form_cov(cam, cfg, c, cS, cE);
+        cut_endpoint(cam, homog, DT_inv, L.Jl, L.sP, L.eP, cS, cE, c0, S7);
+    }
+    asm volatile("" ::: "memory");
+    {
+        LineCovSrc c;
+        double cS[9], cE[9];
+        load_cov_src(Ls, q, c);
+        form_cov(cam, cfg, c, cS, cE);
+        cut_endpoint(cam, homog, DT_inv, L.Jl, L.eP, L.sP, cE, cS, c1, E7);
+    }
+    cut_assemble<true>(S7, E7, info);
+}
+template <bool COV>
+__device__ __forceinline__ void load_line_sel(const KParams& p, const DevLines& L, size_t q, LineCutData& d) {
+    if constexpr (COV) load_line_cov(p.cam, p.cfg, L, q, d);
+    else load_line(L, q, d);
+}
+
 
 template <typename T>
 __device__ __forceinline__ T sym3_t(const T* A, const T* x, const T* y) {
@@ -206,7 +259,7 @@
                     ? 1.0 : 0.0;
 }
 
-template <int W>
+template <int W, bool COV>
 __global__ void __launch_bounds__(64 * W) k_cut_prep(KParams p) {
     extern __shared__ double prep_lds[];
     const int b = blockIdx.x;
@@ -249,7 +302,7 @@
             if (lane < cnt) {
                 if (lines) {
                     LineCutData d;
-                    load_line(L, lb + mls[m], d);
+                    load_line_sel<COV>(p, L, lb + mls[m], d);
                     poseInfoOnLine<false>(cam, homog, Dl, d, 0.0, 0.0, info);
 #pragma unroll
                     for (int i = PD_ERR; i < CUT_FAST; ++i) fd[i] = 0.0;
@@ -1859,6 +1912,7 @@
 #ifndef GFPL_FIN_WAVES
 #define GFPL_FIN_WAVES 4
 #endif
+template <bool COV>
 __global__ void __launch_bounds__(64, GFPL_FIN_WAVES) k_cut_finish(KParams p) {
     const int b = blockIdx.x;
     const int nls = p.tr.n_matched_ls[b];
@@ -1884,16 +1938,23 @@
             r0 = L.cut[2 * q];
             r1 = L.cut[2 * q + 1];
         } else if (live) {
-            load_line(L, q, d);
             r0 = L.cut[2 * q];
             r1 = L.cut[2 * q + 1];
-            poseInfoOnLine<true>(cam, p.cfg.homog_th, Dl, d, r0, r1, info);
+            if constexpr (COV) {
+                load_line_ends(L, q, d);
+                poseInfoOnLine_cov(cam, p.cfg, p.cfg.homog_th, Dl, d, L, q, r0, r1, info);
+            } else {
+                load_line(L, q, d);
+                poseInfoOnLine<true>(cam, p.cfg.homog_th, Dl, d, r0, r1, info);
+            }
             double2* iv = reinterpret_cast<double2*>(L.invcov + 36 * q);
 #pragma unroll
             for (int i = 0; i < 18; ++i) iv[i] = make_double2(info[2 * i], info[2 * i + 1]);
         }
         if (live && !(fabs(r0) < 0.0001 && fabs(r1) < 0.0001)) {
             double sP[3] = {d.sP[0], d.sP[1], d.sP[2]}, eP[3] = {d.eP[0], d.eP[1], d.eP[2]};
+            double fx = cam.fx;
+            if constexpr (COV) asm volatile("" : "+s"(fx));
             if (fabs(r0) > 0.0001) {
                 double s[3];
                 for (int k = 0; k < 3; ++k) s[k] = (1 - r0) * sP[k] + r0 * eP[k];
@@ -1901,7 +1962,7 @@
                 double uv[2];
                 projection(cam, sP, uv);
                 L.spl[2 * q] = uv[0]; L.spl[2 * q + 1] = uv[1];
-                L.sdisp[q] = (cam.fx * cam.b) / sP[2];
+                L.sdisp[q] = (fx * cam.b) / sP[2];
             }
             if (fabs(r1) > 0.0001) {
                 double e[3];
@@ -1910,7 +1971,7 @@
                 double uv[2];
                 projection(cam, eP, uv);
                 L.epl[2 * q] = uv[0]; L.epl[2 * q + 1] = uv[1];
-                L.edisp[q] = (cam.fx * cam.b) / eP[2];
+                L.edisp[q] = (fx * cam.b) / eP[2];
             }
         }
     }
@@ -2604,22 +2665,34 @@
 
 static int cut_prep_w8_max_b() { return env_int("GFPL_CUT_PREP_W8_MAX_B", 256); }
 
-hipError_t launch_line_cut(const KParams& p, hipStream_t s, const hipEvent_t* marks) {
+template <bool COV>
+static hipError_t launch_cut_prep(const KParams& p, hipStream_t s) {
+    if (p.B <= cut_prep_w8_max_b()) {
+        static std::atomic<unsigned long long> attr{0};
+        const hipError_t e =
+            ensure_dyn_lds(reinterpret_cast<const void*>(k_cut_prep<8, COV>), (int)cut_prep_lds(8), &attr);
+        if (e != hipSuccess) return e;
+        hipLaunchKernelGGL(HIP_KERNEL_NAME(k_cut_prep<8, COV>), dim3(p.B), dim3(512), cut_prep_lds(8), s, p);
+    } else {
+        hipLaunchKernelGGL(HIP_KERNEL_NAME(k_cut_prep<1, COV>), dim3(p.B), dim3(64), cut_prep_lds(1), s, p);
+    }
+    return hipSuccess;
+}
+static void launch_cut_finish(const KParams& p, hipStream_t s, bool cov_fresh) {
+    if (cov_fresh) hipLaunchKernelGGL(k_cut_finish<true>, dim3(p.B), dim3(64), 0, s, p);
+    else hipLaunchKernelGGL(k_cut_finish<false>, dim3(p.B), dim3(64), 0, s, p);
+}
+
+hipError_t launch_line_cut(const KParams& p, hipStream_t s, const hipEvent_t* marks, bool cov_fresh) {
     const int mode = p.cfg.cut_proof;
     const dim3 gsearch((p.B + CUT_G - 1) / CUT_G);
-    if (p.B <= cut_prep_w8_max_b()) {
-        static std::atomic<unsigned long long> attr{0};
-        const hipError_t e = ensure_dyn_lds(reinterpret_cast<const void*>(k_cut_prep<8>), (int)cut_prep_lds(8), &attr);
-        if (e != hipSuccess) return e;
-        hipLaunchKernelGGL(k_cut_prep<8>, dim3(p.B), dim3(512), cut_prep_lds(8), s, p);
-    } else {
-        hipLaunchKernelGGL(k_cut_prep<1>, dim3(p.B), dim3(64), cut_prep_lds(1), s, p);
-    }
+    const hipError_t ep = cov_fresh ? launch_cut_prep<true>(p, s) : launch_cut_prep<false>(p, s);
+    if (ep != hipSuccess) return ep;
     if (!p.cfg.cut_with_max_vol) {
         if (marks) (void)hipEventRecord(marks[0], s);
         hipLaunchKernelGGL(k_cut_search_eig, gsearch, dim3(64), 0, s, p);
         if (marks) (void)hipEventRecord(marks[1], s);
-        hipLaunchKernelGGL(k_cut_finish, dim3(p.B), dim3(64), 0, s, p);
+        launch_cut_finish(p, s, cov_fresh);
         return hipGetLastError();
     }
     if (mode == 2) {
@@ -2648,7 +2721,7 @@
         hipLaunchKernelGGL(k_cut_vtab, dim3(p.B), dim3(256), 0, s, p);
         hipLaunchKernelGGL(k_cut_search<true>, gsearch, dim3(64), 0, s, p);
     }
-    hipLaunchKernelGGL(k_cut_finish, dim3(p.B), dim3(64), 0, s, p);
+    launch_cut_finish(p, s, cov_fresh);
     return hipGetLastError();
 }
 
diff --git a/gf-pl-slam_amd/csrc/k_stereo.hip b/gf-pl-slam_amd/csrc/k_stereo.hip
--- a/gf-pl-slam_amd/csrc/k_stereo.hip
+++ b/gf-pl-slam_amd/csrc/k_stereo.hip
@@ -760,20 +760,6 @@
     return true;
 }
 
-__device__ void line_uncertainty(const KParams& p, const double* spl, const double* epl, double sdisp,
-                                 double edisp, const double* le, double* covS, double* covE) {
-    double sdisp_std, edisp_std;
-    if (fabs(le[0]) > 0.15) {
-        sdisp_std = p.cfg.ratio_disp_std * sdisp;
-        edisp_std = p.cfg.ratio_disp_std * edisp;
-    } else {
-        sdisp_std = p.cfg.ratio_disp_std_hor * sdisp;
-        edisp_std = p.cfg.ratio_disp_std_hor * edisp;
-    }
-    covMat2D_3D(p.cam, spl[0], spl[1], 1.0, sdisp, sdisp_std, covS);
-    covMat2D_3D(p.cam, epl[0], epl[1], 1.0, edisp, edisp_std, covE);
-}
-
 __device__ void write_line(const KParams& p, DevLines& C, size_t q, const LineOut& L, int idx, const uint8_t* desc) {
     C.spl[2 * q] = L.spl[0]; C.spl[2 * q + 1] = L.spl[1];
     C.epl[2 * q] = L.epl[0]; C.epl[2 * q + 1] = L.epl[1];
@@ -960,9 +946,8 @@
     if (i < n) {
         const size_t q = (size_t)b * p.kl_cap + i;
         double spl[2] = {L.spl[2 * q], L.spl[2 * q + 1]}, epl[2] = {L.epl[2 * q], L.epl[2 * q + 1]};
-        double le[3] = {L.le[3 * q], L.le[3 * q + 1], L.le[3 * q + 2]};
         double cS[9], cE[9];
-        line_uncertainty(p, spl, epl, L.sdisp[q], L.edisp[q], le, cS, cE);
+        line_uncertainty(p.cam, p.cfg, spl, epl, L.sdisp[q], L.edisp[q], L.le[3 * q], cS, cE);
 #pragma unroll
         for (int k = 0; k < 9; ++k) { cs[9 * threadIdx.x + k] = cS[k]; ce[9 * threadIdx.x + k] = cE[k]; }
     }
diff --git a/gf-pl-slam_amd/gfpl/__init__.py b/gf-pl-slam_amd/gfpl/__init__.py
--- a/gf-pl-slam_amd/gfpl/__init__.py
+++ b/gf-pl-slam_amd/gfpl/__init__.py
@@ -590,6 +590,7 @@
             "gfpl_last_step_counts": ([P, P], C.c_int),
             "gfpl_last_step_track_counts": ([P, P], C.c_int),
             "gfpl_last_step_cut_proof": ([P, P], C.c_int),
+            "gfpl_last_cut_formed_cov": ([P], C.c_int),
             "gfpl_debug_cut_records": ([P, C.c_int, P, C.c_int], C.c_int),
             "gfpl_debug_step_records": ([P, P], C.c_int),
             "gfpl_debug_clocks": ([P, P], C.c_int),
@@ -2187,6 +2188,12 @@
         check(self.L.gfpl_last_step_cut_proof(self.h, v.ctypes.data), "last_step_cut_proof")
         return {"redone": int(v[0]), "steps_proven": int(v[1]), "vref_evals": int(v[2]), "lines": int(v[3])}
 
+    def last_cut_formed_cov(self) -> bool:
+        r = self.L.gfpl_last_cut_formed_cov(self.h)
+        if r < 0:
+            check(r, "last_cut_formed_cov")
+        return bool(r)
+
     def debug_cut_records(self, b: int, n_lines: int) -> np.ndarray:
         out = np.zeros((n_lines, 80), np.float64)
         check(self.L.gfpl_debug_cut_records(self.h, b, out.ctypes.data, n_lines), "debug_cut_records")
diff --git a/include/gfpl.h b/include/gfpl.h
--- a/include/gfpl.h
+++ b/include/gfpl.h
@@ -676,6 +676,7 @@
 int  gfpl_last_step_counts(gfpl_seqbatch* sb, int64_t* counts8);
 int  gfpl_last_step_track_counts(gfpl_seqbatch* sb, int64_t* counts4);
 int  gfpl_last_step_cut_proof(gfpl_seqbatch* sb, int64_t* counts4);
+int  gfpl_last_cut_formed_cov(gfpl_seqbatch* sb);
 int  gfpl_debug_cut_records(gfpl_seqbatch* sb, int b, double* out, int n_lines);
 enum {
     GFPL_STEP_B_STEREO_POINTS = 0,
```

Result: no change. 816,900 (median of 6 runs) (+0.8%).
